# sinamalakouti/CDDMSL

Hardware: AMD Instinct MI355X
Metric: images/sec (train step) VOC+Clipart RN50-C4 (higher is better)
Workload: dtype bf16

## Files before the change

### cddmsl_amd/csrc/conv_fwd.hip

```cpp
#include "gemm_common.h"

namespace {

template <typename T> __device__ __forceinline__ void load8(const char* p, float* f);
template <> __device__ __forceinline__ void load8<__bf16>(const char* p, float* f) {
  const u32x4 v = *(const u32x4*)p;
#pragma unroll
  for (int j = 0; j < 4; ++j) { f[2 * j] = bf2f(v[j] & 0xffff); f[2 * j + 1] = bf2f(v[j] >> 16); }
}
template <> __device__ __forceinline__ void load8<float>(const char* p, float* f) {
  const f32x4 a = ((const f32x4*)p)[0], b = ((const f32x4*)p)[1];
  f[0] = a[0]; f[1] = a[1]; f[2] = a[2]; f[3] = a[3]; f[4] = b[0]; f[5] = b[1]; f[6] = b[2]; f[7] = b[3];
}

__device__ __forceinline__ int swz(int row, int chunk) { return row * KCH + (chunk ^ ((row >> 1) & 7)); }

template <typename T>
__global__ __launch_bounds__(256, 2) void k_conv_fwd_reg(ConvArgs p) {
  __shared__ __attribute__((aligned(16))) u32x4 lds[2][BM * KCH];
  const int t = threadIdx.x;
  const int ntn = (p.Cout + BN - 1) / BN;
  const int tile_n = blockIdx.x % ntn, tile_m = blockIdx.x / ntn;
  const int m0 = tile_m * BM, n0 = tile_n * BN;
  const int cc = t & 7, rb = t >> 3;
// ... 125 lines not shown
#pragma unroll
            for (int j = 0; j < 8; ++j) v[j] = fmaxf(v[j], 0.f);
          }
          if (p.relu_mask) {
            float mv[8];
            load8<T>(p.relu_mask + ((long)m * p.ldm + n) * Mma<T>::ES, mv);
#pragma unroll
            for (int j = 0; j < 8; ++j) if (!(mv[j] > 0.f)) v[j] = 0.f;
          }
          if (p.out_f32 || Mma<T>::ES == 4) {
            f32x4* dst = (f32x4*)(p.y + ((long)m * p.ldy + n) * 4);
            f32x4 o0 = {v[0], v[1], v[2], v[3]}, o1 = {v[4], v[5], v[6], v[7]};
            dst[0] = o0; dst[1] = o1;
          } else {
            u32x4 o = {pack2bf(v[0], v[1]), pack2bf(v[2], v[3]), pack2bf(v[4], v[5]), pack2bf(v[6], v[7])};
            *(u32x4*)(p.y + ((long)m * p.ldy + n) * 2) = o;
          }
        }
      }
    }
    return;
  }
#pragma unroll
  for (int b = 0; b < 2; ++b) {
    int n = n0 + wn * 64 + b * 32 + r;
    if (n >= p.Cout) continue;
    float sc = p.scale ? p.scale[n] : 1.f;
    float bi = p.bias ? p.bias[n] : 0.f;
#pragma unroll
    for (int a = 0; a < 2; ++a) {
#pragma unroll
      for (int g = 0; g < 16; ++g) {
        int m = m0 + wm * 64 + a * 32 + (g & 3) + 8 * (g >> 2) + 4 * h;
        if (m >= p.M) continue;
        float v = affine<T>(acc[a][b][g], sc, bi);
        if (p.residual) v += Mma<T>::load(p.residual + ((long)m * p.ldr + n) * Mma<T>::ES);
        if (p.relu) v = fmaxf(v, 0.f);
        if (p.relu_mask && !(Mma<T>::load(p.relu_mask + ((long)m * p.ldm + n) * Mma<T>::ES) > 0.f)) v = 0.f;
        if (p.out_f32) *(float*)(p.y + ((long)m * p.ldy + n) * 4) = v;
        else Mma<T>::store(p.y + ((long)m * p.ldy + n) * Mma<T>::ES, v);
      }
    }
  }
}


__device__ __forceinline__ long pooled_row(const ConvArgs& p, int m) {
  const unsigned tq = fdiv((unsigned)m, p.dWo), ox = m - tq * p.Wo;
  const unsigned img = fdiv(tq, p.dHo), oy = tq - img * p.Ho;
  const unsigned hp = p.Ho >> 1, wp = p.Wo >> 1;
  return ((oy >> 1) < hp && (ox >> 1) < wp) ? ((long)img * hp + (oy >> 1)) * wp + (ox >> 1) : -1L;
}

template <typename T>
__global__ __launch_bounds__(256, 2) void k_conv_fwd(ConvArgs p) {
  __shared__ __attribute__((aligned(16))) u32x4 lds[2][2][BM * KCH];
  const int t = threadIdx.x;
  p.x += (long)blockIdx.y * p.bx; p.w += (long)blockIdx.y * p.bw; p.y += (long)blockIdx.y * p.by;
  const int wvu = __builtin_amdgcn_readfirstlane(t >> 6);
  const int ntn = (p.Cout + BN - 1) / BN;
  const int lbid = xcd_remap(blockIdx.x, gridDim.x);
  const int tile_n = lbid % ntn, tile_m = lbid / ntn;
  const int m0 = tile_m * BM, n0 = tile_n * BN;
  const int cc = t & 7, rb = t >> 3;
  const int cl = cc ^ ((rb >> 1) & 7);

  long rowoff[4], wrow[4];
  int iy0[4], ix0[4];
  bool vm[4], vn[4];
#pragma unroll
  for (int i = 0; i < 4; ++i) {
    int m = m0 + rb + 32 * i;
    vm[i] = m < p.M;
    unsigned mm = vm[i] ? m : 0;
    unsigned tq = fdiv(mm, p.dWo), ox = mm - tq * p.Wo;
    unsigned img = fdiv(tq, p.dHo), oy = tq - img * p.Ho;
    iy0[i] = (int)oy * p.stride - p.pad;
    ix0[i] = (int)ox * p.stride - p.pad;
    rowoff[i] = ((((long)img * p.Hi + iy0[i]) * p.Wi + ix0[i]) * p.xrs) * 16;
    int n = n0 + rb + 32 * i;
    vn[i] = n < p.Cout;
    wrow[i] = (long)(vn[i] ? n : 0) * p.wrs * 16;
  }
  const int nkt = (p.Kc + KCH - 1) / KCH;
  const char* zp = (const char*)g_zero_page;
  const bool taps = !(p.KH == 1 && p.KW == 1 && p.pad == 0);
  int kc = cl;
  int pp0 = (int)fdiv((unsigned)kc, p.dcpp);
  int coff = kc - pp0 * p.cpp;
  int ky = (int)fdiv((unsigned)pp0, p.dKW), kx = pp0 - ky * p.KW;

  const bool fast = (p.cpp & 7) == 0;
  const char* pa[4];
  const char* pb[4];
  int inca[4], incb[4];
  int tiles_left_in_tap = 0;
  auto retap = [&]() {
    const int delta = ((ky * p.Wi + kx) * p.xrs + coff) * 16;
#pragma unroll
    for (int i = 0; i < 4; ++i) {
      bool ok = vm[i];
      if (taps) {
        int iy = iy0[i] + ky, ix = ix0[i] + kx;
        ok = ok && iy >= 0 && iy < p.Hi && ix >= 0 && ix < p.Wi;
      }
      pa[i] = ok ? p.x + rowoff[i] + delta : zp;
      inca[i] = ok ? KCH * 16 : 0;
    }
  };
  if (fast) {
#pragma unroll
    for (int i = 0; i < 4; ++i) {
      pb[i] = vn[i] ? p.w + wrow[i] + (long)kc * 16 : zp;
      incb[i] = vn[i] ? KCH * 16 : 0;
// ... 344 lines not shown
          *(unsigned short*)(ob + row * (NT * 64) + (nt * 32 + r) * 2) = f2bf(v);
        }
#pragma unroll
      for (int i = 0; i < 2 * NT; ++i) {
        const u32x4 o = *(const u32x4*)(ob + (i * 64 + lane) * 16);
        __builtin_amdgcn_raw_buffer_store_b128(o, ry, (unsigned)((i * 64 + lane) * 16), tile * (32 * NT * 64), 0);
      }
      continue;
    }
    const unsigned vy = (unsigned)(((tile * 32 + 4 * hh) * p.ldy + r) * ES), vmk = (unsigned)(((tile * 32 + 4 * hh) * p.ldm + r) * ES);
#pragma unroll
    for (int nt = 0; nt < NT; ++nt)
#pragma unroll
      for (int g = 0; g < 16; ++g) {
        const int row = (g & 3) + 8 * (g >> 2);
        float v = affine<T>(acc[nt][g], sc[nt], bi[nt]);
        asm("v_max_f32 %0, %1, %2" : "=v"(v) : "v"(v), "s"(relu_floor));
        if (p.relu_mask) {
          float mv;
          if (ES == 2) mv = bf2f((unsigned)__builtin_amdgcn_raw_buffer_load_b16(rm, vmk, (row * p.ldm + nt * 32) * ES, 0));
          else mv = __builtin_bit_cast(float, __builtin_amdgcn_raw_buffer_load_b32(rm, vmk, (row * p.ldm + nt * 32) * ES, 0));
          if (!(mv > 0.f)) v = 0.f;
        }
        if (ES == 2) __builtin_amdgcn_raw_buffer_store_b16((unsigned short)f2bf(v), ry, vy, (row * p.ldy + nt * 32) * ES, 0);
        else __builtin_amdgcn_raw_buffer_store_b32(__builtin_bit_cast(unsigned, v), ry, vy, (row * p.ldy + nt * 32) * ES, 0);
      }
  }
}

template <typename T> void launch_small(const ConvArgs& a, unsigned nb, hipStream_t st) {
  if (a.KH == 1 && a.cpp == 8) hipLaunchKernelGGL((k_conv3x3_small<T, 8, 2, 1>), dim3(nb), dim3(256), 0, st, a);
  else if (a.KH == 1) hipLaunchKernelGGL((k_conv3x3_small<T, 32, 2, 1>), dim3(nb), dim3(256), 0, st, a);
  else if (a.cpp == 1 && a.Cout == 32) hipLaunchKernelGGL((k_conv3x3_small<T, 1, 1>), dim3(nb), dim3(256), 0, st, a);
  else if (a.cpp == 1) hipLaunchKernelGGL((k_conv3x3_small<T, 1, 2>), dim3(nb), dim3(256), 0, st, a);
  else if (a.cpp == 8) hipLaunchKernelGGL((k_conv3x3_small<T, 8, 2>), dim3(nb), dim3(256), 0, st, a);
  else if (a.Cout == 32) hipLaunchKernelGGL((k_conv3x3_small<T, 4, 1>), dim3(nb), dim3(256), 0, st, a);
  else if (a.pool_out) {
    if constexpr (sizeof(T) == 2) hipLaunchKernelGGL((k_conv3x3_small<T, 4, 2, 9, true>), dim3(nb), dim3(256), 0, st, a);
  }
  else hipLaunchKernelGGL((k_conv3x3_small<T, 4, 2>), dim3(nb), dim3(256), 0, st, a);
}

template <typename T> void launch_tile128(const ConvArgs& a, const Plan& p, hipStream_t st) {
  const dim3 grid(p.gx, p.gy);
  switch (p.kernel) {
    case 8: launch_small<T>(a, p.gx, st); break;
    case 2: hipLaunchKernelGGL(k_conv_fwd_reg<T>, grid, dim3(256), 0, st, a); break;
    default: hipLaunchKernelGGL(k_conv_fwd<T>, grid, dim3(256), 0, st, a); break;
  }
}

}

void launch_fwd_tile128(const ConvArgs& a, const Plan& p, Operand op, hipStream_t st) {
  if (op == OP_BF16) launch_tile128<__bf16>(a, p, st);
  else launch_tile128<float>(a, p, st);
}
```

### cddmsl_amd/csrc/conv_fwd256.hip

```cpp
#include "gemm_common.h"
#include <type_traits>

namespace {

__device__ __forceinline__ unsigned pack4_e4m3(float a, float b, float c, float d) {
  a = __builtin_amdgcn_fmed3f(a, -448.f, 448.f); b = __builtin_amdgcn_fmed3f(b, -448.f, 448.f);
  c = __builtin_amdgcn_fmed3f(c, -448.f, 448.f); d = __builtin_amdgcn_fmed3f(d, -448.f, 448.f);
  int w = __builtin_amdgcn_cvt_pk_fp8_f32(a, b, 0, false);
  w = __builtin_amdgcn_cvt_pk_fp8_f32(c, d, w, true);
  return (unsigned)w;
}

struct fp8e4 { unsigned char v; };
template <> struct Mma<fp8e4> {
  static constexpr int ES = 2;
  __device__ static __forceinline__ void step2(f32x16& acc, const u32x4& a0, const u32x4& a1, const u32x4& b0, const u32x4& b1) {
    const i32x8 a = {(int)a0[0], (int)a0[1], (int)a0[2], (int)a0[3], (int)a1[0], (int)a1[1], (int)a1[2], (int)a1[3]};
    const i32x8 b = {(int)b0[0], (int)b0[1], (int)b0[2], (int)b0[3], (int)b1[0], (int)b1[1], (int)b1[2], (int)b1[3]};
    acc = __builtin_amdgcn_mfma_scale_f32_32x32x64_f8f6f4(a, b, acc, 0, 0, 0, 0x7f7f7f7f, 0, 0x7f7f7f7f);
  }
};
template <typename T> struct MmaQuad {
  __device__ static __forceinline__ void run(f32x16& c0, f32x16& c1, const u32x4 (*fa)[4], const u32x4* fb) {
#pragma unroll
// ... 152 lines not shown
#pragma unroll
      for (int j = 0; j < 8; ++j) asm("v_max_f32 %0, %1, %2" : "=v"(v[j]) : "v"(v[j]), "s"(relu_floor));
      if (has_msk) {
        float mv[8];
        if (ES == 2) {
#pragma unroll
          for (int j = 0; j < 4; ++j) { mv[2 * j] = bf2f(rmsk_[i][0][j] & 0xffff); mv[2 * j + 1] = bf2f(rmsk_[i][0][j] >> 16); }
        } else {
#pragma unroll
          for (int j = 0; j < 4; ++j) {
            mv[j] = __builtin_bit_cast(f32x4, rmsk_[i][0])[j]; mv[4 + j] = __builtin_bit_cast(f32x4, rmsk_[i][ES / 2 - 1])[j];
          }
        }
#pragma unroll
        for (int j = 0; j < 8; ++j) if (!(mv[j] > 0.f)) v[j] = 0.f;
      }
      const unsigned so = (unsigned)((a * 32 + 8 * i) * p.ldy * eso);
      if (emit8) {
#pragma unroll
        for (int j = 0; j < 8; ++j) am8 = absmax_bits(am8, v[j]);
        const u32x2 o8 = {pack4_e4m3(v[0] * q8s, v[1] * q8s, v[2] * q8s, v[3] * q8s), pack4_e4m3(v[4] * q8s, v[5] * q8s, v[6] * q8s, v[7] * q8s)};
        __builtin_amdgcn_raw_buffer_store_b64(o8, ry8, vy8, (unsigned)((a * 32 + 8 * i) * p.ldy), CDDMSL_STORE_AUX);
        asm volatile("s_nop 4" ::: "memory");
        asm volatile("" :: "v"(o8));
      }
      if (f32out) {
        const u32x4 o0 = {__builtin_bit_cast(unsigned, v[0]), __builtin_bit_cast(unsigned, v[1]), __builtin_bit_cast(unsigned, v[2]), __builtin_bit_cast(unsigned, v[3])};
        const u32x4 o1 = {__builtin_bit_cast(unsigned, v[4]), __builtin_bit_cast(unsigned, v[5]), __builtin_bit_cast(unsigned, v[6]), __builtin_bit_cast(unsigned, v[7])};
        __builtin_amdgcn_raw_buffer_store_b128(o0, ry, vy, so, CDDMSL_STORE_AUX);
        __builtin_amdgcn_raw_buffer_store_b128(o1, ry, vy, so + 16, CDDMSL_STORE_AUX);
        asm volatile("s_nop 4" ::: "memory");
        asm volatile("" :: "v"(o0), "v"(o1));
      } else {
        const u32x4 o = {pack2bf(v[0], v[1]), pack2bf(v[2], v[3]), pack2bf(v[4], v[5]), pack2bf(v[6], v[7])};
        if (p.nt_out) __builtin_amdgcn_raw_buffer_store_b128(o, ry, vy, so, CDDMSL_STORE_AUX);
        else __builtin_amdgcn_raw_buffer_store_b128(o, ry, vy, so, 0);
        asm volatile("s_nop 4" ::: "memory");
        asm volatile("" :: "v"(o));
      }
    }
    if (DEPTH == 2 && a + 2 < 4 && !rf32) fetch(a + 2, rresb[a % DEPTH], rmskb[a % DEPTH]);
  };
  put(std::integral_constant<int, 0>{});
  pass(std::integral_constant<int, 0>{});
  pass(std::integral_constant<int, 1>{});
  pass(std::integral_constant<int, 2>{});
  pass(std::integral_constant<int, 3>{});
  if (emit8 && p.amax8) {
    am8 = wave_max_u(am8);
    if (lane == 0) atomicMax(p.amax8 + (blockIdx.x & 63), am8);
  }
}

template <typename T, bool TAPS, bool RPOOL = false, int EPI = -1, bool PERSIST = false, bool SPLITK = false>
__global__ __launch_bounds__(512) void k_conv_fwd256(ConvArgs p) {
  __shared__ __attribute__((aligned(16))) u32x4 lds[2 * 2 * 2 * 128 * KCH];
  const int t_in = threadIdx.x;
  p.x += (long)blockIdx.y * p.bx; p.w += (long)blockIdx.y * p.bw; p.y += (long)blockIdx.y * p.by;
  const int ntn = p.Cout >> 8;
  const int ntiles = PERSIST ? (p.tile_limit ? p.tile_limit : ntn * ((p.M + 255) >> 8)) : 0;
  int lbid = PERSIST ? (int)((blockIdx.x & 7) * (gridDim.x >> 3) + (blockIdx.x >> 3))
           : SPLITK ? p.tile0 + (int)(blockIdx.x / (unsigned)p.ksplits) : xcd_remap(blockIdx.x, gridDim.x);
  const int kt0 = SPLITK ? (int)(blockIdx.x % (unsigned)p.ksplits) * p.kper : 0;
  if (PERSIST && lbid >= ntiles) return;
  for (;;) {
  int t = t_in;
  if (PERSIST) asm volatile("" : "+v"(t));
  const int lane = t & 63;
#ifdef CDDMSL_TILE_STAMPS
  const unsigned long long ts_entry = __builtin_amdgcn_s_memrealtime();
#endif
  const int wvu = __builtin_amdgcn_readfirstlane(t >> 6);
  const int wr = wvu >> 2, wc = wvu & 3;
  const int tile_n = lbid % ntn, tile_m = lbid / ntn;
  const int m0 = tile_m * 256, n0 = tile_n * 256;
  const int cl = (t & 7) ^ ((t >> 4) & 7);
  const int nkt = SPLITK ? min(p.kper, (p.Kc >> 3) - kt0) : (p.Kc >> 3);
  const int tpt = p.cpp >> 3;

  auto rowoff = [&](int m, int& iy0, int& ix0) {
    const unsigned tq = fdiv((unsigned)m, p.dWo), ox = m - tq * p.Wo;
    const unsigned img = fdiv(tq, p.dHo), oy = tq - img * p.Ho;
    iy0 = (int)oy * p.stride - p.pad; ix0 = (int)ox * p.stride - p.pad;
    return (((long)img * p.Hi + iy0) * p.Wi + ix0) * p.xrs * 16;
  };
  int iyb, ixb;
  const long base_a = rowoff(m0, iyb, ixb);
  const __amdgpu_buffer_rsrc_t ra_rsrc = __builtin_amdgcn_make_buffer_rsrc((void*)(p.x + base_a), 0, 0x7fffffff, 0x00020000);
  const __amdgpu_buffer_rsrc_t rb_rsrc = __builtin_amdgcn_make_buffer_rsrc((void*)(p.w + (long)n0 * p.wrs * 16), 0, 0x7fffffff, 0x00020000);
  unsigned va[2][2], vinv[2][2], vb[2][2];
  int iy0[2][2], ix0[2][2];
#pragma unroll
  for (int h = 0; h < 2; ++h)
#pragma unroll
    for (int i = 0; i < 2; ++i) {
      const int m = m0 + i * 128 + h * 64 + (t >> 3);
      const bool vm = m < p.M;
      const long ro = rowoff(vm ? m : m0, iy0[h][i], ix0[h][i]);
      va[h][i] = (unsigned)(ro - base_a) + cl * 16;
      if (!vm) { iy0[h][i] = -(1 << 20); if (!TAPS) va[h][i] |= 0x80000000u; }
      vinv[h][i] = 0;
      vb[h][i] = (unsigned)(((2 * i + (t >> 8)) * 64 + h * 32 + ((t >> 3) & 31)) * p.wrs + cl) * 16;
    }
  if (TAPS) {
    unsigned xm[2][2] = {{0, 0}, {0, 0}};
    for (int kx = 0; kx < p.KW; ++kx)
#pragma unroll
      for (int h = 0; h < 2; ++h)
#pragma unroll
        for (int i = 0; i < 2; ++i) xm[h][i] |= ((unsigned)(ix0[h][i] + kx) >= (unsigned)p.Wi ? 1u : 0u) << kx;
    const unsigned full = (1u << p.KW) - 1u;
    for (int ky = 0; ky < p.KH; ++ky)
#pragma unroll
      for (int h = 0; h < 2; ++h)
#pragma unroll
        for (int i = 0; i < 2; ++i) vinv[h][i] |= ((unsigned)(iy0[h][i] + ky) >= (unsigned)p.Hi ? full : xm[h][i]) << (ky * p.KW);
  }
  const int step_col = (p.xrs - (p.cpp - KCH)) * 16;
// ... 126 lines not shown
    readA(I1{}, fa1);
    flipA();
    if (more2) {
      stageB(I0{}, d);
      asm volatile("s_waitcnt vmcnt(4)" ::: "memory");
    } else if (more1) {
      asm volatile("s_waitcnt vmcnt(0)" ::: "memory");
    } else if (PREF) {
      const bool is_res = (EPI & 1) != 0;
      const char* base = is_res ? p.residual : p.relu_mask;
      const int ld = is_res ? p.ldr : p.ldm;
      long bytes = ((long)p.M - m0) * ld * 2;
      if (bytes > 0x7fffffffL) bytes = 0x7fffffffL;
      const __amdgpu_buffer_rsrc_t rs = __builtin_amdgcn_make_buffer_rsrc((void*)(base + (long)m0 * ld * 2), 0, (int)bytes, 0x00020000);
      const unsigned vo = (unsigned)(((wr * 128 + (lane >> 3)) * ld + n0 + wc * 64 + (lane & 7) * 8) * 2);
#pragma unroll
      for (int a = 0; a < 2; ++a)
#pragma unroll
        for (int i = 0; i < 4; ++i) pre[a][i] = __builtin_amdgcn_raw_buffer_load_b128(rs, vo, (a * 32 + 8 * i) * ld * 2, 0);
    }
    CDDMSL_PHASE_SYNC_IN();
    CDDMSL_MMA_QUAD(1, 1, fa1, fb1);
    CDDMSL_PHASE_SYNC_OUT(1, 1);
    if (more1) readA(I0{}, fa0);
    if (more2) stageB(I1{}, d);
    if (last && !SPLITK) {
      const int n = n0 + wc * 64 + (lane & 7) * 8;
      const f32x4 one = {1.f, 1.f, 1.f, 1.f}, zero = {0.f, 0.f, 0.f, 0.f};
      sb[0] = p.scale ? *(const f32x4*)(p.scale + n) : one; sb[1] = p.scale ? *(const f32x4*)(p.scale + n + 4) : one;
      sb[2] = p.bias ? *(const f32x4*)(p.bias + n) : zero; sb[3] = p.bias ? *(const f32x4*)(p.bias + n + 4) : zero;
    }
    CDDMSL_PHASE_SYNC_IN();
    CDDMSL_MMA_QUAD(1, 0, fa1, fb0);
    CDDMSL_PHASE_SYNC_OUT(1, 0);
  };
  for (int kt = 0; kt + 1 < nkt; ++kt) ktile(kt, std::false_type{});
  ktile(nkt - 1, std::true_type{});
  if (wr == 0) __builtin_amdgcn_s_barrier();
#ifdef CDDMSL_TILE_STAMPS
  const unsigned long long ts_epi = __builtin_amdgcn_s_memrealtime();
#endif
#undef CDDMSL_MMA_QUAD
#undef CDDMSL_PHASE_SYNC_IN
#undef CDDMSL_PHASE_SYNC_OUT

  if (SPLITK) {
    store_frags((f32x4*)p.partial + (long)blockIdx.x * (8 * 32 * 64) + (wvu * 32) * 64 + lane, acc);
    return;
  }
  tile_epilogue<T, RPOOL, EPI, PREF>(p, acc, (float*)lds + wvu * 4096, wr, wc, lane, m0, n0, pre, sb);
#ifdef CDDMSL_TILE_STAMPS
  if (p.tstamps && lane == 0) {
    if (!PERSIST) asm volatile("s_waitcnt vmcnt(0)" ::: "memory");
    unsigned long long* o = p.tstamps + ((long)(PERSIST ? lbid : (int)blockIdx.x) * 8 + wvu) * 4;
    o[0] = ts_entry; o[1] = ts_loop; o[2] = ts_epi; o[3] = __builtin_amdgcn_s_memrealtime();
  }
#endif
  if (!PERSIST) break;
  lbid += gridDim.x;
  if (lbid >= ntiles) break;
  __builtin_amdgcn_s_barrier();
  }
}

template <typename T, bool TAPS, int EPI>
__global__ __launch_bounds__(256, 2) void k_conv_fwd2(ConvArgs p) {
  constexpr int SA = 256 * 64, SB = 128 * 64, SS = SA + SB, STAGES = 3;
  __shared__ __attribute__((aligned(16))) u32x4 lds[STAGES * SS / 16];
  const int t = threadIdx.x, lane = t & 63;
#ifdef CDDMSL_TILE_STAMPS
  const unsigned long long ts_entry = __builtin_amdgcn_s_memrealtime();
#endif
  p.x += (long)blockIdx.y * p.bx; p.w += (long)blockIdx.y * p.bw; p.y += (long)blockIdx.y * p.by;
  const int wvu = __builtin_amdgcn_readfirstlane(t >> 6);
  const int wr = wvu >> 1, wc = wvu & 1;
  const int ntn = p.Cout >> 7;
  const int lbid = xcd_remap(blockIdx.x, gridDim.x);
  const int tile_n = lbid % ntn, tile_m = lbid / ntn;
  const int m0 = tile_m * 256, n0 = tile_n * 128;
  const int cl = (t & 3) ^ ((t >> 3) & 3);
  const int nkt = p.Kc >> 2;
  const int tpt = p.cpp >> 2;

  auto rowoff = [&](int m, int& iy0, int& ix0) {
    const unsigned tq = fdiv((unsigned)m, p.dWo), ox = m - tq * p.Wo;
    const unsigned img = fdiv(tq, p.dHo), oy = tq - img * p.Ho;
    iy0 = (int)oy * p.stride - p.pad; ix0 = (int)ox * p.stride - p.pad;
    return (((long)img * p.Hi + iy0) * p.Wi + ix0) * p.xrs * 16;
  };
  int iyb, ixb;
  const long base_a = rowoff(m0, iyb, ixb);
  const __amdgpu_buffer_rsrc_t ra_rsrc = __builtin_amdgcn_make_buffer_rsrc((void*)(p.x + base_a), 0, 0x7fffffff, 0x00020000);
  const __amdgpu_buffer_rsrc_t rb_rsrc = __builtin_amdgcn_make_buffer_rsrc((void*)(p.w + (long)n0 * p.wrs * 16), 0, 0x7fffffff, 0x00020000);
  unsigned va[4], vinv[4], vb[2];
  int iy0[4], ix0[4];
#pragma unroll
  for (int i = 0; i < 4; ++i) {
    const int m = m0 + (t >> 2) + 64 * i;
    const bool vm = m < p.M;
    const long ro = rowoff(vm ? m : m0, iy0[i], ix0[i]);
    va[i] = (unsigned)(ro - base_a) + cl * 16;
    if (!vm) { iy0[i] = -(1 << 20); if (!TAPS) va[i] |= 0x80000000u; }
    vinv[i] = 0;
  }
#pragma unroll
  for (int i = 0; i < 2; ++i) vb[i] = (unsigned)((((t >> 2) + 64 * i) * p.wrs + cl) * 16);
  if (TAPS) {
    unsigned xm[4] = {0, 0, 0, 0};
    for (int kx = 0; kx < p.KW; ++kx)
#pragma unroll
      for (int i = 0; i < 4; ++i) xm[i] |= ((unsigned)(ix0[i] + kx) >= (unsigned)p.Wi ? 1u : 0u) << kx;
    const unsigned full = (1u << p.KW) - 1u;
    for (int ky = 0; ky < p.KH; ++ky)
#pragma unroll
      for (int i = 0; i < 4; ++i) vinv[i] |= ((unsigned)(iy0[i] + ky) >= (unsigned)p.Hi ? full : xm[i]) << (ky * p.KW);
  }
  const int step_col = (p.xrs - (p.cpp - 4)) * 16;
  const int step_row = ((p.Wi - (p.KW - 1)) * p.xrs - (p.cpp - 4)) * 16;
  int left = tpt, tap = 0, kxs = 0;
  unsigned soa = 0, sob = 0;

  char* const L = (char*)lds;
  auto stage = [&](int st) {
    char* dst = L + st * SS + wvu * 1024;
#pragma unroll
    for (int i = 0; i < 4; ++i) {
      unsigned v = va[i];
      if (TAPS) v |= __builtin_amdgcn_ubfe(vinv[i], (unsigned)tap, 1u) << 31;
      blds16(ra_rsrc, v, soa, dst + i * 4096);
    }
// ... 157 lines not shown
  S = (nktot + kper - 1) / kper;
  if (S < 2 || rem * S * 65536 * 4 > ws_bytes) return {};
  return {rem, (int)S, kper};
}

template <typename T, bool TAPS> void launch256_main(const ConvArgs& a, dim3 grid, hipStream_t st, int epi) {
  if constexpr (std::is_same<T, __bf16>::value && !TAPS) {
    const int nb = persistent_blocks();
    if (nb > 0 && grid.y == 1 && (int)grid.x > nb && (a.Kc >> 3) <= env_int("CDDMSL_PERSIST_MAXKT", 8)) {
      with_epi(epi, [&](auto e) { hipLaunchKernelGGL((k_conv_fwd256<T, false, false, decltype(e)::value, true>), dim3(nb), dim3(512), 0, st, a); });
      return;
    }
  }
  with_epi(epi, [&](auto e) { hipLaunchKernelGGL((k_conv_fwd256<T, TAPS, false, decltype(e)::value>), grid, dim3(512), 0, st, a); });
}

template <typename T, bool TAPS> void launch256(const ConvArgs& a, dim3 grid, hipStream_t st, void* ws, long ws_bytes) {
  const int epi = epi_of(a);
  if (sizeof(T) == 4 || epi < 0) { hipLaunchKernelGGL((k_conv_fwd256<T, TAPS, false, -1>), grid, dim3(512), 0, st, a); return; }
  if constexpr (sizeof(T) != 4) {
    if constexpr (std::is_same<T, __bf16>::value) {
      const int tiles = (int)grid.x;
      const TailSplit ts = grid.y == 1 ? plan_tail_split(tiles, persistent_blocks_raw(), a.Kc >> 3, ws ? ws_bytes : 0) : TailSplit{};
      if (ts.splits) {
        ConvArgs m = a, t = a;
        m.tile_limit = tiles - ts.rem;
        launch256_main<T, TAPS>(m, dim3((unsigned)(tiles - ts.rem), 1), st, epi);
        t.partial = (float*)ws; t.tile0 = tiles - ts.rem; t.ksplits = ts.splits; t.kper = ts.kper;
        hipLaunchKernelGGL((k_conv_fwd256<T, TAPS, false, -1, false, true>), dim3((unsigned)(ts.rem * ts.splits)), dim3(512), 0, st, t);
        hipLaunchKernelGGL(k_conv_split_reduce, dim3((unsigned)(ts.rem * 64)), dim3(256), 0, st, t);
        return;
      }
    }
    launch256_main<T, TAPS>(a, grid, st, epi);
  }
}

template <typename T> void launch_tile256(const ConvArgs& a, const Plan& p, hipStream_t st, void* ws, long ws_bytes) {
  const dim3 grid(p.gx, p.gy);
  const bool taps = !(a.KH == 1 && a.KW == 1 && a.pad == 0);
  if constexpr (std::is_same<T, fp8e4>::value) {
    if (taps) launch256<T, true>(a, grid, st, ws, ws_bytes);
    else launch256<T, false>(a, grid, st, ws, ws_bytes);
  } else if (p.kernel == 11) {
    if (taps) launch_fwd2<T, true>(a, grid, st);
    else launch_fwd2<T, false>(a, grid, st);
  } else {
    if (a.res_pool) hipLaunchKernelGGL((k_conv_fwd256<T, false, true>), grid, dim3(512), 0, st, a);
    else if (taps) launch256<T, true>(a, grid, st, ws, ws_bytes);
    else launch256<T, false>(a, grid, st, ws, ws_bytes);
  }
}

}

void launch_fwd_tile256(const ConvArgs& a, const Plan& p, Operand op, hipStream_t st, void* ws, long ws_bytes) {
  if (op == OP_BF16) launch_tile256<__bf16>(a, p, st, ws, ws_bytes);
  else if (op == OP_F32) launch_tile256<float>(a, p, st, ws, ws_bytes);
  else launch_tile256<fp8e4>(a, p, st, ws, ws_bytes);
}
```

### cddmsl_amd/csrc/conv_wgrad.hip

```cpp
#include "gemm_common.h"

namespace {

template <typename T> struct TrFrag;
template <> struct TrFrag<__bf16> {
  __device__ static __forceinline__ u32x4 read(const u32x4* base, int mrow0, int col0, int lane) {
    int g = lane >> 4, li = lane & 15, q = li >> 2, pp = li & 3;
    int hh = g >> 1;
    int col = col0 + 16 * (g & 1) + 4 * pp;
    const char* b = (const char*)base;
    const char* a0 = b + (long)(mrow0 + 8 * hh + q) * (WROW * 16) + col * 2;
    const char* a1 = a0 + 4 * (WROW * 16);
    i16x4 v0 = __builtin_amdgcn_ds_read_tr16_b64_v4i16((__attribute__((address_space(3))) i16x4*)a0);
    i16x4 v1 = __builtin_amdgcn_ds_read_tr16_b64_v4i16((__attribute__((address_space(3))) i16x4*)a1);
    u32x2 p0 = __builtin_bit_cast(u32x2, v0), p1 = __builtin_bit_cast(u32x2, v1);
    u32x4 r = {p0[0], p0[1], p1[0], p1[1]};
    return r;
  }
  static constexpr int MSTEP = 16;
};
template <> struct TrFrag<float> {
  __device__ static __forceinline__ u32x4 read(const u32x4* base, int mrow0, int col0, int lane) {
    int r = lane & 31, hh = lane >> 5;
    const char* b = (const char*)base;
// ... 113 lines not shown
}


template <typename T> struct TrFragS;
template <> struct TrFragS<__bf16> {
  struct Off { int o0, o1; };
  __device__ static __forceinline__ Off prep(int col0, int lane) {
    int g = lane >> 4, li = lane & 15, q = li >> 2, pp = li & 3;
    int hh = g >> 1;
    int ch = ((col0 + 16 * (g & 1)) >> 3) + (pp >> 1);
    int r0 = 8 * hh + q, r1 = r0 + 4;
    Off o;
    o.o0 = r0 * 256 + 16 * (ch ^ fsw(r0)) + 8 * (pp & 1);
    o.o1 = r1 * 256 + 16 * (ch ^ fsw(r1)) + 8 * (pp & 1);
    return o;
  }
  __device__ static __forceinline__ u32x4 read(const u32x4* base, int ms, const Off& o) {
    const unsigned a = (unsigned)(size_t)(const __attribute__((address_space(3))) char*)((const char*)base) + ms * 256;
    u32x2 p0, p1;
    asm volatile("ds_read_b64_tr_b16 %0, %1" : "=v"(p0) : "v"(a + o.o0));
    asm volatile("ds_read_b64_tr_b16 %0, %1" : "=v"(p1) : "v"(a + o.o1));
    u32x4 r = {p0[0], p0[1], p1[0], p1[1]};
    return r;
  }
  static constexpr int MSTEP = 16;
};
template <> struct TrFragS<float> {
  struct Off { int o[4]; };
  __device__ static __forceinline__ Off prep(int col0, int lane) {
    int r = lane & 31, hh = lane >> 5;
    int byte = (col0 + r) * 4;
    Off o;
#pragma unroll
    for (int j = 0; j < 4; ++j) {
      int row = 4 * hh + j;
      o.o[j] = row * 256 + (byte & 15) + 16 * (byte >> 4);
    }
    return o;
  }
  __device__ static __forceinline__ u32x4 read(const u32x4* base, int ms, const Off& o) {
    const char* b = (const char*)base;
    u32x4 v;
#pragma unroll
    for (int j = 0; j < 4; ++j) {
      int off = o.o[j] + ms * 256;
      int row = off >> 8, ch = (off >> 4) & 15;
      v[j] = *(const unsigned int*)(b + (off & ~0xf0) + 16 * (ch ^ fsw(row)));
    }
    return v;
  }
  static constexpr int MSTEP = 8;
};

template <typename T>
__global__ __launch_bounds__(256, 2) void k_conv_wgrad_dma(WgradArgs p) {
  constexpr int ES = Mma<T>::ES;
  constexpr int COLS = 256 / ES;
  __shared__ __attribute__((aligned(16))) u32x4 lds[2][2][WM * 16];
  const int t = threadIdx.x, lane = t & 63, wv = t >> 6;
  p.x += (long)blockIdx.y * p.bx; p.dy += (long)blockIdx.y * p.bd;
  char* outp = (char*)p.dw + (long)blockIdx.y * p.bo;
  const int wvu = __builtin_amdgcn_readfirstlane(t >> 6);
  const int ntn = (p.Cout + COLS - 1) / COLS, ntk = (p.K + COLS - 1) / COLS;
  int bid = xcd_remap(blockIdx.x, gridDim.x);
  const int tile_k = bid % ntk; bid /= ntk;
  const int tile_n = bid % ntn; bid /= ntn;
  const int split = bid;
  const int n0 = tile_n * COLS, k0 = tile_k * COLS;
  const int mt0 = split * p.mtiles_per_split;
  const int total_mt = (p.M + WM - 1) / WM;
  const int mt1 = min(mt0 + p.mtiles_per_split, total_mt);

  const int cc = t & 15, rb = t >> 4;
  const int cl = cc ^ fsw(rb);
  const int kc = k0 * ES / 16 + cl;
  const bool vk = kc < p.Kc;
  const int pp = vk ? kc / p.cpp : 0, coff = vk ? kc - pp * p.cpp : 0;
  const int ky = pp / p.KW, kx = pp - ky * p.KW;
  const int nc = n0 * ES / 16 + cl;
  const bool vn = nc < p.ncc;
  const bool taps = !(p.KH == 1 && p.KW == 1);
  const char* zp = (const char*)g_zero_page;

  int m[4];
  const char* pd[4];
  const char* px[4];
#pragma unroll
  for (int i = 0; i < 4; ++i) {
    m[i] = mt0 * WM + rb + 16 * i;
    pd[i] = p.dy + ((long)m[i] * p.ldd) * ES + (long)nc * 16;
    px[i] = p.x + (((long)m[i] + (long)(ky - p.pad) * p.Wi + (kx - p.pad)) * p.xrs) * 16 + (long)coff * 16;
  }
  const long dstep = (long)WM * p.ldd * ES, xstep = (long)WM * p.xrs * 16;

  auto stage = [&](int buf) {
#pragma unroll
    for (int i = 0; i < 4; ++i) {
      bool vmm = m[i] < p.M;
      glds16((vmm && vn) ? pd[i] : zp, &lds[buf][0][(4 * wvu + 16 * i) * 16]);
    }
#pragma unroll
    for (int i = 0; i < 4; ++i) {
      bool ok = (m[i] < p.M) & vk;
      if (taps) {
        unsigned mm = min((unsigned)m[i], (unsigned)(p.M - 1));
        unsigned tq = fdiv(mm, p.dWo);
        unsigned ox = mm - tq * p.Wo;
        unsigned oy = tq - fdiv(tq, p.dHo) * p.Ho;
        ok = ok & ((unsigned)((int)oy - p.pad + ky) < (unsigned)p.Hi) & ((unsigned)((int)ox - p.pad + kx) < (unsigned)p.Wi);
      }
      glds16(ok ? px[i] : zp, &lds[buf][1][(4 * wvu + 16 * i) * 16]);
    }
#pragma unroll
    for (int i = 0; i < 4; ++i) { m[i] += WM; pd[i] += dstep; px[i] += xstep; }
  };

  constexpr int WT = COLS / 2;
  constexpr int NT = WT / 32;
  const int wn = wv >> 1, wk = wv & 1;
  f32x16 acc[NT][NT];
#pragma unroll
  for (int a = 0; a < NT; ++a)
#pragma unroll
    for (int b = 0; b < NT; ++b)
#pragma unroll
      for (int r = 0; r < 16; ++r) acc[a][b][r] = 0.f;

  typename TrFragS<T>::Off offa[NT], offb[NT];
#pragma unroll
  for (int i = 0; i < NT; ++i) {
    offa[i] = TrFragS<T>::prep(wn * WT + i * 32, lane);
    offb[i] = TrFragS<T>::prep(wk * WT + i * 32, lane);
  }

  if (mt0 < mt1) stage(0);
  for (int mt = mt0; mt < mt1; ++mt) {
    const int cur = (mt - mt0) & 1;
    if (mt + 1 < mt1) {
      stage(cur ^ 1);
      asm volatile("s_waitcnt vmcnt(8)" ::: "memory");
    } else {
      asm volatile("s_waitcnt vmcnt(0)" ::: "memory");
    }
    __builtin_amdgcn_s_barrier();
#pragma unroll
    for (int ms = 0; ms < WM; ms += TrFragS<T>::MSTEP) {
      u32x4 fa[NT], fb[NT];
#pragma unroll
      for (int i = 0; i < NT; ++i) {
        fa[i] = TrFragS<T>::read(lds[cur][0], ms, offa[i]);
        fb[i] = TrFragS<T>::read(lds[cur][1], ms, offb[i]);
      }
      asm volatile("s_waitcnt lgkmcnt(0)" ::: "memory");
      __builtin_amdgcn_sched_barrier(0);
#pragma unroll
      for (int a = 0; a < NT; ++a)
#pragma unroll
        for (int b = 0; b < NT; ++b) Mma<T>::step(acc[a][b], fa[a], fb[b]);
    }
    asm volatile("s_waitcnt lgkmcnt(0)" ::: "memory");
    __builtin_amdgcn_s_barrier();
  }

  const int r = lane & 31, h = lane >> 5;
  if (p.ws) {
    f32x4* dst = (f32x4*)p.ws + ((long)(split * ntn + tile_n) * ntk + tile_k) * (4 * NT * NT * 4 * 64) + (wv * NT * NT * 4) * 64 + lane;
#pragma unroll
    for (int a = 0; a < NT; ++a)
#pragma unroll
      for (int b = 0; b < NT; ++b)
#pragma unroll
        for (int g4 = 0; g4 < 4; ++g4) {
          const f32x4 v = {acc[a][b][4 * g4], acc[a][b][4 * g4 + 1], acc[a][b][4 * g4 + 2], acc[a][b][4 * g4 + 3]};
          dst[((a * NT + b) * 4 + g4) * 64] = v;
        }
    return;
  }
#pragma unroll
  for (int a = 0; a < NT; ++a)
#pragma unroll
    for (int b = 0; b < NT; ++b) {
      int k = k0 + wk * WT + b * 32 + r;
      if (k >= p.K) continue;
#pragma unroll
      for (int g = 0; g < 16; ++g) {
        int n = n0 + wn * WT + a * 32 + (g & 3) + 8 * (g >> 2) + 4 * h;
        if (n >= p.Cout) continue;
        float v = acc[a][b][g] * (p.scale ? p.scale[n] : 1.f);
        long o = (long)n * p.ldo + k;
        if (p.direct == 0) atomicAdd((float*)outp + o, v);
        else if (p.direct == 1) ((float*)outp)[o] = v;
        else Mma<T>::store(outp + o * ES, v);
      }
    }
}

template <typename T>
__global__ __launch_bounds__(256, 2) void k_gemm_tn_stream(WgradArgs p, int nbatch, int bpb) {
  constexpr int ES = Mma<T>::ES;
  constexpr int COLS = 256 / ES;
  __shared__ __attribute__((aligned(16))) u32x4 lds[2][2][WM * 16];
  const int t = threadIdx.x, lane = t & 63, wv = t >> 6;
  const int wvu = __builtin_amdgcn_readfirstlane(t >> 6);
  const int ntk = (p.K + COLS - 1) / COLS;
  const int tile_k = blockIdx.x % ntk, tile_n = blockIdx.x / ntk;
  const int n0 = tile_n * COLS, k0 = tile_k * COLS;
  const int b0 = blockIdx.y * bpb, nb = min(bpb, nbatch - b0);
  const int nmt = (p.M + WM - 1) / WM;
  const int nit = nb * nmt;

  const int cc = t & 15, rb = t >> 4;
  const int cl = cc ^ fsw(rb);
  const int kc = k0 * ES / 16 + cl, nc = n0 * ES / 16 + cl;
  const bool vk = kc < p.Kc, vn = nc < p.ncc;
  const char* zp = (const char*)g_zero_page;
  int sb = 0, smt = 0;
  auto stage = [&](int buf) {
    const char* db = p.dy + (long)(b0 + sb) * p.bd + (long)nc * 16;
    const char* xb = p.x + (long)(b0 + sb) * p.bx + (long)kc * 16;
// ... 218 lines not shown
        for (int g = 0; g < 16; ++g) {
          const int n0 = a * 32 + (g & 3) + 8 * (g >> 2);
          const bool exists = a * 4 + (g >> 2) < NG;
          const bool lo_ok = n0 >= 1 && n0 <= P, hi_ok = n0 + 4 >= 1 && n0 + 4 <= P;
          if (exists) {
            const int n = n0 + 4 * h;
            const float v = acc[a][g];
            gacc[a][g] += (n == 0) ? t0 : v;
            if (lo_ok || hi_ok) {
              if (h ? hi_ok : lo_ok) {
                const unsigned word = (n - 1) < 32 ? mlo : mhi;
                const bool keep = (word >> ((n - 1) & 31)) & 1u;
                Mma<__bf16>::store(outp + ((long)(n - 1) * p.ldo + k) * 2, keep ? v + base : 0.f);
              }
            }
          }
          acc[a][g] = 0.f;
        }
      return;
    }
#pragma unroll
    for (int a = 0; a < NTN; ++a)
#pragma unroll
      for (int g = 0; g < 16; ++g) {
        if (a * 4 + (g >> 2) < NG) {
          const int n = a * 32 + (g & 3) + 8 * (g >> 2) + 4 * h;
          const float v = acc[a][g];
          const long o = (long)n * p.ldo + k;
          if (MODE == 0) atomicAdd((float*)outp + o, v);
          else if (MODE == 1) ((float*)outp)[o] = v;
          else Mma<__bf16>::store(outp + o * 2, v);
        }
        acc[a][g] = 0.f;
      }
  };
  {
    int it = 0;
    for (; it + 2 < nit; ++it) item(it, std::integral_constant<int, 2>{});
    if (it + 1 < nit) { item(it, std::integral_constant<int, 1>{}); ++it; }
    if (it < nit) item(it, std::integral_constant<int, 0>{});
  }
  if (MODE == 3 && p.gpos) {
    const int k = k0 + wvu * 32 + r;
#pragma unroll
    for (int a = 0; a < NTN; ++a)
#pragma unroll
      for (int g = 0; g < 16; ++g) {
        const int n = a * 32 + (g & 3) + 8 * (g >> 2) + 4 * h;
        if (a * 4 + (g >> 2) < NG && n <= P) atomicAdd(p.gpos + (long)n * p.K + k, gacc[a][g]);
      }
  }
}

__global__ __launch_bounds__(512) void k_wgrad256(WgradArgs p) {
  __shared__ __attribute__((aligned(16))) u32x4 lds[2 * 2 * 2 * 64 * 16];
  const int t = threadIdx.x, lane = t & 63;
#ifdef CDDMSL_TILE_STAMPS
  const unsigned long long ts_entry = __builtin_amdgcn_s_memrealtime();
  unsigned long long ts_loop = ts_entry;
#endif
  p.x += (long)blockIdx.y * p.bx; p.dy += (long)blockIdx.y * p.bd;
  char* outp = (char*)p.dw + (long)blockIdx.y * p.bo;
  const int wvu = __builtin_amdgcn_readfirstlane(t >> 6);
  const int wn = wvu >> 2, wk = wvu & 3;
  const int ntn = p.Cout >> 8, ntk = p.K >> 8;
  int bid = xcd_remap(blockIdx.x, gridDim.x);
  const int tile_k = bid % ntk; bid /= ntk;
  const int tile_n = bid % ntn; bid /= ntn;
  const int n0 = tile_n * 256, k0 = tile_k * 256;
  const int mt0 = bid * p.mtiles_per_split;
  const int nmt = min(p.mtiles_per_split, (p.M + WM - 1) / WM - mt0);
  const bool taps = !(p.KH == 1 && p.KW == 1);

  const int rb = t >> 4, cl = (t & 15) ^ fsw(rb);
  const int gd = (cl >> 3) * 16 + (cl & 7);
  const int gx = (cl >> 2) * 8 + (cl & 3);
  const int kc = (k0 >> 3) + gx;
  const int pp = kc / p.cpp, coff = kc - pp * p.cpp;
  const int ky = pp / p.KW, kx = pp - ky * p.KW;
  unsigned vd[2], vx[2];
#pragma unroll
  for (int i = 0; i < 2; ++i) {
    vd[i] = (unsigned)((i * 32 + rb) * p.ldd * 2 + gd * 16);
    vx[i] = (unsigned)((((i * 32 + rb) + ky * p.Wi + kx) * p.xrs + coff) * 16);
  }
  const __amdgpu_buffer_rsrc_t rd = __builtin_amdgcn_make_buffer_rsrc((void*)(p.dy + ((long)mt0 * WM * p.ldd + n0) * 2), 0, 0x80000000u, 0x00020000);
  const __amdgpu_buffer_rsrc_t rx = __builtin_amdgcn_make_buffer_rsrc((void*)(p.x + ((long)mt0 * WM - p.pad * p.Wi - p.pad) * p.xrs * 16), 0, 0x80000000u, 0x00020000);
  const unsigned dstep = (unsigned)(WM * p.ldd * 2), xstep = (unsigned)(WM * p.xrs * 16);
  const int mrow = mt0 * WM + rb;

  char* const L = (char*)lds;
  auto stageD = [&](auto H, int buf, int T) {
    constexpr int h = decltype(H)::value;
    char* dst = L + (buf << 16) + (h << 14) + wvu * 1024;
#pragma unroll
    for (int i = 0; i < 2; ++i) {
      const unsigned inv = (mrow + T * WM + i * 32 < p.M) ? 0u : 0x80000000u;
      __builtin_amdgcn_raw_ptr_buffer_load_lds(rd, (__attribute__((address_space(3))) void*)(dst + i * 8192 - h * 128), 16,
                                               (int)(vd[i] | inv), (int)(T * dstep), h * 128, 0);
    }
  };
  unsigned xinv[2];
  auto validX = [&](int T) {
#pragma unroll
    for (int i = 0; i < 2; ++i) {
      const int m = mrow + T * WM + i * 32;
      bool ok = m < p.M;
      if (taps) {
        const unsigned mm = min((unsigned)m, (unsigned)(p.M - 1));
        const unsigned tq = fdiv(mm, p.dWo);
        const unsigned ox = mm - tq * p.Wo;
        const unsigned oy = tq - fdiv(tq, p.dHo) * p.Ho;
        ok = ok & ((unsigned)((int)oy - p.pad + ky) < (unsigned)p.Hi) & ((unsigned)((int)ox - p.pad + kx) < (unsigned)p.Wi);
      }
      xinv[i] = ok ? 0u : 0x80000000u;
    }
  };
  auto stageX = [&](auto J, int buf, int T) {
    constexpr int j = decltype(J)::value;
    char* dst = L + (buf << 16) + (1 << 15) + (j << 14) + wvu * 1024;
#pragma unroll
// ... 82 lines not shown
#ifdef CDDMSL_TILE_STAMPS
    ts_loop = __builtin_amdgcn_s_memrealtime();
#endif

    for (int kt = 0; kt < nmt; ++kt) {
      const int d = kt & 1;
      const bool more1 = kt + 1 < nmt, more2 = kt + 2 < nmt;
      CDDMSL_READ_B(0, fb0)
      if (more1) stageD(I1{}, d ^ 1, kt + 1);
      CDDMSL_PHASE_SYNC_IN(CDDMSL_WAIT4(fb0))
      CDDMSL_MMA_QUAD(0, 0, fa0, fb0);
      CDDMSL_PHASE_SYNC_OUT(0, 0)
      CDDMSL_READ_B(1, fb1)
      CDDMSL_FLIP_B()
      if (more2) { stageD(I0{}, d, kt + 2); validX(kt + 2); }
      CDDMSL_PHASE_SYNC_IN(CDDMSL_WAIT4(fb1))
      CDDMSL_MMA_QUAD(0, 1, fa0, fb1);
      CDDMSL_PHASE_SYNC_OUT(0, 1)
      CDDMSL_READ_A(1, fa1)
      CDDMSL_FLIP_A()
      if (more2) {
        stageX(I0{}, d, kt + 2);
        asm volatile("s_waitcnt vmcnt(4)" ::: "memory");
      } else {
        asm volatile("s_waitcnt vmcnt(0)" ::: "memory");
      }
      CDDMSL_PHASE_SYNC_IN(CDDMSL_WAIT8(fa1))
      CDDMSL_MMA_QUAD(1, 1, fa1, fb1);
      CDDMSL_PHASE_SYNC_OUT(1, 1)
      if (more1) { CDDMSL_READ_A(0, fa0) }
      if (more2) stageX(I1{}, d, kt + 2);
      CDDMSL_PHASE_SYNC_IN(CDDMSL_WAIT8(fa0))
      CDDMSL_MMA_QUAD(1, 0, fa1, fb0);
      CDDMSL_PHASE_SYNC_OUT(1, 0)
    }
    if (wn == 0) __builtin_amdgcn_s_barrier();
  }
#undef CDDMSL_TR2
#undef CDDMSL_WAIT4
#undef CDDMSL_WAIT8
#undef CDDMSL_READ_A
#undef CDDMSL_READ_B
#undef CDDMSL_FLIP_A
#undef CDDMSL_FLIP_B
#undef CDDMSL_MMA_QUAD
#undef CDDMSL_PHASE_SYNC_IN
#undef CDDMSL_PHASE_SYNC_OUT

#ifdef CDDMSL_TILE_STAMPS
  const unsigned long long ts_epi = __builtin_amdgcn_s_memrealtime();
#endif
  const int r = lane & 31, h = lane >> 5;
  if (p.ws) {
    store_frags((f32x4*)p.ws + ((long)(bid * ntn + tile_n) * ntk + tile_k) * (8 * 32 * 64) + (wvu * 32) * 64 + lane, acc);
  } else
#pragma unroll
  for (int a = 0; a < 4; ++a)
#pragma unroll
    for (int b = 0; b < 2; ++b) {
      const int k = k0 + wk * 64 + b * 32 + r;
#pragma unroll
      for (int g = 0; g < 16; ++g) {
        const int n = n0 + wn * 128 + a * 32 + (g & 3) + 8 * (g >> 2) + 4 * h;
        const float v = acc[a][b][g] * (p.scale ? p.scale[n] : 1.f);
        const long o = (long)n * p.ldo + k;
        if (p.direct == 0) atomicAdd((float*)outp + o, v);
        else if (p.direct == 1) ((float*)outp)[o] = v;
        else Mma<__bf16>::store(outp + o * 2, v);
      }
    }
#ifdef CDDMSL_TILE_STAMPS
  if (p.tstamps && lane == 0) {
    asm volatile("s_waitcnt vmcnt(0)" ::: "memory");
    unsigned long long* o = p.tstamps + ((long)blockIdx.x * 8 + wvu) * 4;
    o[0] = ts_entry; o[1] = ts_loop; o[2] = ts_epi; o[3] = __builtin_amdgcn_s_memrealtime();
  }
#endif
}

__global__ __launch_bounds__(512) void k_wgrad256_f8(WgradArgs p) {
  __shared__ __attribute__((aligned(16))) u32x4 lds[4 * 2 * 64 * 16];
  const int t = threadIdx.x, lane = t & 63;
  const int wvu = __builtin_amdgcn_readfirstlane(t >> 6);
  const int wn = wvu >> 2, wk = wvu & 3;
  const int ntn = p.Cout >> 8, ntk = p.K >> 8;
  int bid = xcd_remap(blockIdx.x, gridDim.x);
  const int tile_k = bid % ntk; bid /= ntk;
  const int tile_n = bid % ntn; bid /= ntn;
  const int n0 = tile_n * 256, k0 = tile_k * 256;
  const int mt0 = bid * p.mtiles_per_split;
  const int nmt_real = min(p.mtiles_per_split, (p.M + WM - 1) / WM - mt0);
  const int nmt = (nmt_real + 1) & ~1;
  const int mlim = min(p.M, (mt0 + nmt_real) * WM);
  const bool taps = !(p.KH == 1 && p.KW == 1);

  const int rq = lane >> 4, r8 = (wvu & 1) * 4 + rq;
  const int cl = (lane & 15) ^ (r8 << 1);
  const int pp = k0 / p.Cin, coff = (k0 - pp * p.Cin) >> 4;
  const int ky = pp / p.KW, kx = pp - ky * p.KW;
  unsigned vd[2], vx[2];
#pragma unroll
  for (int i = 0; i < 2; ++i) {
    const int row = i * 32 + wvu * 4 + rq;
    vd[i] = (unsigned)(row * p.ldd + cl * 16);
    vx[i] = (unsigned)(((row + ky * p.Wi + kx) * p.xrs + coff + cl) * 16);
  }
  const __amdgpu_buffer_rsrc_t rd = __builtin_amdgcn_make_buffer_rsrc((void*)(p.dy + ((long)mt0 * WM * p.ldd + n0)), 0, 0x80000000u, 0x00020000);
// ... 135 lines not shown
#pragma unroll
      for (int g = 0; g < 16; ++g) {
        const int n = n0 + wn * 128 + a * 32 + (g & 3) + 8 * (g >> 2) + 4 * h;
        atomicAdd(p.dw + (long)n * p.ldo + k, acc[a][b][g] * (p.scale ? p.scale[n] : 1.f));
      }
    }
}

}

template <int WAVES, int FR>
__global__ __launch_bounds__(256) void k_wgrad_reduce(const f32x4* ws, float* dw, const float* scale, int ntn, int ntk, int splits, int Cout, int K, int ldo) {
  constexpr int SLOTS = WAVES * FR * 64;
  constexpr int TN = WAVES == 8 ? 256 : 128;
  const int tile = blockIdx.x / (SLOTS / 256), q = (blockIdx.x % (SLOTS / 256)) * 256 + threadIdx.x;
  const int tile_k = tile % ntk, tile_n = tile / ntk;
  const long ntiles = (long)ntn * ntk;
  const f32x4* src = ws + (long)tile * SLOTS + q;
  f32x4 sum = {0.f, 0.f, 0.f, 0.f};
  int s = 0;
  for (; s + 4 <= splits; s += 4) {
    const f32x4 a = src[(s + 0) * ntiles * SLOTS], b = src[(s + 1) * ntiles * SLOTS], c = src[(s + 2) * ntiles * SLOTS], d = src[(s + 3) * ntiles * SLOTS];
    sum += (a + b) + (c + d);
  }
  for (; s < splits; ++s) sum += src[s * ntiles * SLOTS];
  const int wv = q / (FR * 64), j = (q / 64) % FR, lane = q & 63, r = lane & 31, h = lane >> 5, g4 = j & 3;
  int a, b, wn, wk;
  if (WAVES == 8) { a = j >> 3; b = (j >> 2) & 1; wn = wv >> 2; wk = wv & 3; }
  else { a = j >> 3; b = (j >> 2) & 1; wn = wv >> 1; wk = wv & 1; }
  const int n = tile_n * TN + wn * (WAVES == 8 ? 128 : 64) + a * 32 + 8 * g4 + 4 * h;
  const int k = tile_k * TN + wk * 64 + b * 32 + r;
  if (k >= K) return;
#pragma unroll
  for (int e = 0; e < 4; ++e)
    if (n + e < Cout) dw[(long)(n + e) * ldo + k] += sum[e] * (scale ? scale[n + e] : 1.f);
}

static bool use_workspace(long blocks, long tile_floats, void* ws, long ws_bytes) {
  if (env_int("CDDMSL_WGRAD_WS", 1) == 0) return false;
  return ws != nullptr && blocks * tile_floats * 4 <= ws_bytes;
}

template <int WAVES, int FR>
static void launch_wgrad_split(void (*kernel)(WgradArgs), WgradArgs& a, const Plan& p, hipStream_t st, void* wsp, long ws_bytes) {
  constexpr int TN = WAVES == 8 ? 256 : 128, SLOTS = WAVES * FR * 64;
  const int ntn = (a.Cout + TN - 1) / TN, ntk = (a.K + TN - 1) / TN;
  const bool ws = p.splits > 1 && use_workspace((long)p.gx, SLOTS * 4, wsp, ws_bytes);
  if (ws) a.ws = (float*)wsp;
  hipLaunchKernelGGL(kernel, dim3(p.gx), dim3(WAVES * 64), 0, st, a);
  if (ws) hipLaunchKernelGGL((k_wgrad_reduce<WAVES, FR>), dim3((unsigned)(ntn * ntk * (SLOTS / 256))), dim3(256), 0, st, (const f32x4*)wsp, a.dw, a.scale,
                             ntn, ntk, p.splits, a.Cout, a.K, a.ldo);
}

void launch_wgrad(WgradArgs& a, const Plan& p, Operand op, hipStream_t st, void* ws, long ws_bytes) {
  switch (p.kernel) {
    case 12: launch_wgrad_split<8, 32>(k_wgrad256_f8, a, p, st, ws, ws_bytes); break;
    case 6: launch_wgrad_split<8, 32>(k_wgrad256, a, p, st, ws, ws_bytes); break;
    case 5:
      if (op == OP_BF16) launch_wgrad_split<4, 16>(k_conv_wgrad_dma<__bf16>, a, p, st, ws, ws_bytes);
      else hipLaunchKernelGGL(k_conv_wgrad_dma<float>, dim3(p.gx), dim3(256), 0, st, a);
      break;
    default:
      if (op == OP_BF16) hipLaunchKernelGGL(k_conv_wgrad<__bf16>, dim3(p.gx), dim3(256), 0, st, a);
      else hipLaunchKernelGGL(k_conv_wgrad<float>, dim3(p.gx), dim3(256), 0, st, a);
  }
}

void launch_gemm_tn(const WgradArgs& p, Operand op, const Plan& pl, int batch, int mode, hipStream_t st) {
  const dim3 grid(pl.gx, pl.gy);
  if (pl.kernel == 9) {
#define CDDMSL_TNS(NG)                                                                                              \
  case NG:                                                                                                          \
    if (mode == 0) hipLaunchKernelGGL((k_gemm_tn_small<NG, 0>), grid, dim3(256), 0, st, p, batch, pl.bpb);      \
    else if (mode == 1) hipLaunchKernelGGL((k_gemm_tn_small<NG, 1>), grid, dim3(256), 0, st, p, batch, pl.bpb); \
    else hipLaunchKernelGGL((k_gemm_tn_small<NG, 2>), grid, dim3(256), 0, st, p, batch, pl.bpb);                \
    break;
    switch (p.Cout / 8) { CDDMSL_TNS(1) CDDMSL_TNS(2) CDDMSL_TNS(3) CDDMSL_TNS(4) CDDMSL_TNS(5) CDDMSL_TNS(6) CDDMSL_TNS(7) CDDMSL_TNS(8) }
#undef CDDMSL_TNS
  } else if (pl.kernel == 7) {
    if (op == OP_BF16) hipLaunchKernelGGL(k_gemm_tn_stream<__bf16>, grid, dim3(256), 0, st, p, batch, pl.bpb);
    else hipLaunchKernelGGL(k_gemm_tn_stream<float>, grid, dim3(256), 0, st, p, batch, pl.bpb);
  } else {
    if (op == OP_BF16) hipLaunchKernelGGL(k_conv_wgrad_dma<__bf16>, grid, dim3(256), 0, st, p);
    else hipLaunchKernelGGL(k_conv_wgrad_dma<float>, grid, dim3(256), 0, st, p);
  }
}

void launch_attnpool_dx(const WgradArgs& p, unsigned gx, unsigned gy, int nbatch, int bpb, hipStream_t st) {
  hipLaunchKernelGGL((k_gemm_tn_small<7, 3, 49>), dim3(gx, gy), dim3(256), 0, st, p, nbatch, bpb);
}
```

### cddmsl_amd/csrc/gemm_common.h

```cpp
#pragma once
#include "common.h"
#include <cstdlib>

namespace {

constexpr int BM = 128, BN = 128, KCH = 8;

struct FastDiv {
  unsigned mul, shr, d;
};
static inline FastDiv make_fastdiv(unsigned d) {
  FastDiv f;
  f.d = d;
  unsigned s = 0;
  while ((1ull << s) < d) ++s;
  f.shr = s;
  f.mul = (unsigned)(((1ull << 32) * ((1ull << s) - d)) / d + 1);
  return f;
}
__device__ __forceinline__ unsigned fdiv(unsigned n, const FastDiv& f) { return (__umulhi(n, f.mul) + n) >> f.shr; }

template <typename T> __device__ __forceinline__ float affine(float v, float sc, float bi) {
  return sizeof(T) <= 2 ? __builtin_fmaf(v, sc, bi) : v * sc + bi;
}

#ifndef CDDMSL_STORE_AUX
#define CDDMSL_STORE_AUX 2
#endif
#ifndef CDDMSL_LOAD_AUX
#define CDDMSL_LOAD_AUX 0
#endif

struct ConvArgs {
  const char* x;
  const char* w;
  char* y;
  const float* scale;
  const float* bias;
  const char* residual;
  const char* relu_mask;
  int Nimg, Hi, Wi, Cin, Ho, Wo, Cout, KH, KW, stride, pad;
  int ldy, ldr, ldm;
  int relu, out_f32, pool;
  int res_f32;
  int res_pool;
  int M, Kc, cpp;
  FastDiv dWo, dHo, dcpp, dKW;
  int xrs, wrs;
  long bx, bw, by;
  char* y8 = nullptr;
  const float* q8 = nullptr;
  unsigned* amax8 = nullptr;
  float* partial = nullptr;
  int tile0 = 0, ksplits = 1, kper = 0, tile_limit = 0;
  int pool_out = 0;
  FastDiv dWp = {}, dHp = {};
  int nt_out = 1;
#ifdef CDDMSL_TILE_STAMPS
  unsigned long long* tstamps = nullptr;
#endif
};

template <typename T> struct Mma;
template <> struct Mma<__bf16> {
  static constexpr int ES = 2;
  __device__ static __forceinline__ void step(f32x16& acc, const u32x4& a, const u32x4& b) {
    acc = __builtin_amdgcn_mfma_f32_32x32x16_bf16(__builtin_bit_cast(bf16x8, a), __builtin_bit_cast(bf16x8, b), acc, 0, 0, 0);
  }
  __device__ static __forceinline__ float load(const char* p) { return bf2f(*(const unsigned short*)p); }
  __device__ static __forceinline__ void store(char* p, float v) { *(unsigned short*)p = f2bf(v); }
};
template <> struct Mma<float> {
  static constexpr int ES = 4;
  __device__ static __forceinline__ void step(f32x16& acc, const u32x4& a, const u32x4& b) {
    const f32x4 fa = __builtin_bit_cast(f32x4, a), fb = __builtin_bit_cast(f32x4, b);
    acc = __builtin_amdgcn_mfma_f32_32x32x2f32(fa[0], fb[0], acc, 0, 0, 0);
    acc = __builtin_amdgcn_mfma_f32_32x32x2f32(fa[1], fb[1], acc, 0, 0, 0);
    acc = __builtin_amdgcn_mfma_f32_32x32x2f32(fa[2], fb[2], acc, 0, 0, 0);
    acc = __builtin_amdgcn_mfma_f32_32x32x2f32(fa[3], fb[3], acc, 0, 0, 0);
  }
  __device__ static __forceinline__ float load(const char* p) { return *(const float*)p; }
  __device__ static __forceinline__ void store(char* p, float v) { *(float*)p = v; }
};
typedef __attribute__((ext_vector_type(8))) int i32x8;

__device__ __forceinline__ int xcd_remap(int bid, int nblk) {
  const int q = nblk >> 3, rem = nblk & 7, x = bid & 7, j = bid >> 3;
  return (x < rem ? x * (q + 1) : rem * (q + 1) + (x - rem) * q) + j;
}

template <typename T> __device__ __forceinline__ u32x4 avg4(const u32x4& a, const u32x4& b, const u32x4& c, const u32x4& d);
template <> __device__ __forceinline__ u32x4 avg4<float>(const u32x4& a, const u32x4& b, const u32x4& c, const u32x4& d) {
  const f32x4 fa = __builtin_bit_cast(f32x4, a), fb = __builtin_bit_cast(f32x4, b);
  const f32x4 fc = __builtin_bit_cast(f32x4, c), fd = __builtin_bit_cast(f32x4, d);
  f32x4 r = ((fa + fb) + (fc + fd)) * 0.25f;
  return __builtin_bit_cast(u32x4, r);
}
template <> __device__ __forceinline__ u32x4 avg4<__bf16>(const u32x4& a, const u32x4& b, const u32x4& c, const u32x4& d) {
  u32x4 r;
#pragma unroll
  for (int j = 0; j < 4; ++j) {
    float lo = (bf2f(a[j] & 0xffff) + bf2f(b[j] & 0xffff)) + (bf2f(c[j] & 0xffff) + bf2f(d[j] & 0xffff));
    float hi = (bf2f(a[j] >> 16) + bf2f(b[j] >> 16)) + (bf2f(c[j] >> 16) + bf2f(d[j] >> 16));
    r[j] = pack2bf(lo * 0.25f, hi * 0.25f);
  }
  return r;
}

__device__ __attribute__((aligned(16))) unsigned int g_zero_page[4] = {0u, 0u, 0u, 0u};

__device__ __forceinline__ void glds16(const void* g, void* l) {
  __builtin_amdgcn_global_load_lds((const __attribute__((address_space(1))) void*)g,
                                   (__attribute__((address_space(3))) void*)l, 16, 0, 0);
}

struct WgradArgs {
  const char* x;
  const char* dy;
  float* dw;
  const float* scale;
  int Nimg, Hi, Wi, Cin, Ho, Wo, Cout, KH, KW, stride, pad, ldd, pool;
  int M, Kc, cpp, K, ncc;
  int mtiles_per_split;
  FastDiv dWo, dHo;
  int xrs;
  int ldo;
  int direct;
  long bx, bd, bo;
  const float* g0 = nullptr;
  const unsigned long long* mbits = nullptr;
  float* gpos = nullptr;
  float* ws = nullptr;
#ifdef CDDMSL_TILE_STAMPS
  unsigned long long* tstamps = nullptr;
#endif
};

constexpr int WM = 64;
constexpr int WROW = 16 + 4;

__device__ __forceinline__ int fsw(int row) { return ((row & 3) << 2) | ((row >> 2) & 3); }

__device__ __forceinline__ void store_frags(f32x4* dst, const f32x16 (&acc)[4][2]) {
#pragma unroll
  for (int a = 0; a < 4; ++a)
#pragma unroll
    for (int b = 0; b < 2; ++b)
#pragma unroll
      for (int g4 = 0; g4 < 4; ++g4) {
        const f32x4 v = {acc[a][b][4 * g4], acc[a][b][4 * g4 + 1], acc[a][b][4 * g4 + 2], acc[a][b][4 * g4 + 3]};
        dst[((a * 2 + b) * 4 + g4) * 64] = v;
      }
}

static long env_int(const char* name, long dflt, bool* set = nullptr) {
  const char* e = getenv(name);
  if (set) *set = e != nullptr;
  return e ? atol(e) : dflt;
}

enum Operand { OP_BF16 = 0, OP_F32 = 1, OP_FP8 = 2 };
static int elem_size(Operand op) { return op == OP_BF16 ? 2 : op == OP_F32 ? 4 : 1; }

struct Plan {
  int kernel;
  unsigned gx, gy;
  int splits;
  int mtiles_per_split;
  int bpb;
};

static int persistent_blocks_raw() {
  static int ncu = -1;
  if (ncu < 0) {
    int dev = 0, n = 0;
    if (hipGetDevice(&dev) != hipSuccess || hipDeviceGetAttribute(&n, hipDeviceAttributeMultiprocessorCount, dev) != hipSuccess) n = 0;
    ncu = (n / 8) * 8;
  }
  return ncu;
}

}

extern "C" {
__attribute__((visibility("hidden"))) void launch_fwd_tile128(const ConvArgs& a, const Plan& p, Operand op, hipStream_t st);
__attribute__((visibility("hidden"))) void launch_fwd_tile256(const ConvArgs& a, const Plan& p, Operand op, hipStream_t st, void* ws, long ws_bytes);
__attribute__((visibility("hidden"))) void launch_wgrad(WgradArgs& a, const Plan& p, Operand op, hipStream_t st, void* ws, long ws_bytes);
__attribute__((visibility("hidden"))) void launch_gemm_tn(const WgradArgs& p, Operand op, const Plan& pl, int batch, int mode, hipStream_t st);
__attribute__((visibility("hidden"))) void launch_attnpool_dx(const WgradArgs& p, unsigned gx, unsigned gy, int nbatch, int bpb, hipStream_t st);
__attribute__((visibility("hidden"))) bool record_kernel(int id);
}
```

### cddmsl_amd/csrc/gemm_conv.hip

```cpp
#include "gemm_common.h"

namespace {

template <typename T>
__device__ __forceinline__ void weight_prep_body(const float* w, const float* scale, char* wf, char* wd, int Cout, int KH, int KW, int Cin,
                                                 long first, long stride) {
  __shared__ float tile[32][33];
  const int taps = KH * KW, nit = (Cin + 31) / 32, nct = (Cout + 31) / 32;
  const long ntiles = (long)nct * taps * nit;
  const int tx = threadIdx.x & 31, ty = threadIdx.x >> 5;
  constexpr int ES = Mma<T>::ES;
  for (long tl = first; tl < ntiles; tl += stride) {
    const int it = (int)(tl % nit); const long q = tl / nit;
    const int tap = (int)(q % taps), ct = (int)(q / taps);
    const int ky = tap / KW, kx = tap % KW;
    __syncthreads();
#pragma unroll
    for (int r = 0; r < 4; ++r) {
      const int co = ct * 32 + ty + 8 * r, ci = it * 32 + tx;
      float v = 0.f;
      if (co < Cout && ci < Cin) {
        const long i = ((long)co * taps + tap) * Cin + ci;
        v = w[i];
        if (wf) Mma<T>::store(wf + i * ES, v);
// ... 117 lines not shown
  if ((Cin * es) % 16 != 0) return CDDMSL_ERR_ARG;
  if (pool && (KH != 1 || KW != 1 || pad != 0 || stride != 1)) return CDDMSL_ERR_ARG;
  a.x = (const char*)x; a.w = (const char*)w; a.y = (char*)y; a.scale = scale; a.bias = bias;
  a.residual = (const char*)residual; a.relu_mask = (const char*)relu_mask;
  a.Nimg = Nimg; a.Hi = Hi; a.Wi = Wi; a.Cin = Cin; a.Cout = Cout; a.KH = KH; a.KW = KW; a.stride = stride; a.pad = pad;
  if (pool) { a.Ho = Hi / 2; a.Wo = Wi / 2; }
  else { a.Ho = (Hi + 2 * pad - KH) / stride + 1; a.Wo = (Wi + 2 * pad - KW) / stride + 1; }
  if (a.Ho <= 0 || a.Wo <= 0) return CDDMSL_ERR_ARG;
  if ((out_f32 & 2) && (!(out_f32 & 1) || !residual || relu_mask || pool)) return CDDMSL_ERR_ARG;
  a.ldy = ldy; a.ldr = ldr; a.ldm = ldm; a.relu = relu; a.out_f32 = out_f32 & 1; a.pool = pool;
  a.res_f32 = (op == OP_BF16 && (out_f32 & 2)) ? 1 : 0;
  a.res_pool = (out_f32 & 4) ? 1 : 0;
  if (a.res_pool && (!residual || (out_f32 & 2) || pool || KH != 1 || KW != 1 || pad != 0 || (long)Nimg * (a.Ho / 2) * (a.Wo / 2) * ldr * es >= (1L << 31) ||
                     (Cout & 7) || (ldy & 7) || (ldr & 7) || (relu_mask && (ldm & 7)))) return CDDMSL_ERR_ARG;
  if (a.res_f32 && ((Cout & 7) || (ldy & 7) || (ldr & 7))) return CDDMSL_ERR_ARG;
  long M = (long)Nimg * a.Ho * a.Wo;
  if (M > 0x7fffff00L) return CDDMSL_ERR_ARG;
  a.M = (int)M; a.cpp = Cin * es / 16; a.Kc = KH * KW * a.cpp;
  a.dWo = make_fastdiv((unsigned)a.Wo); a.dHo = make_fastdiv((unsigned)a.Ho);
  a.dcpp = make_fastdiv((unsigned)a.cpp); a.dKW = make_fastdiv((unsigned)KW);
  a.xrs = a.cpp; a.wrs = a.Kc; a.bx = a.bw = a.by = 0;
#ifdef CDDMSL_TILE_STAMPS
  a.tstamps = g_tile_stamps;
#endif
  if (a.M == 0) return CDDMSL_OK;
  a.nt_out = nt_out_for((long)a.M * Cout * 2);
  if (y8) {
    if (op == OP_F32 || (out_f32 & 1) || ldy != Cout) return CDDMSL_ERR_ARG;
    a.y8 = (char*)y8; a.q8 = q8; a.amax8 = (unsigned*)amax8;
  }
  return CDDMSL_OK;
}

static int conv_fwd_any(Operand op, const void* x, const void* w, void* y, const float* scale, const float* bias,
                        const void* residual, const void* relu_mask, int Nimg, int Hi, int Wi, int Cin,
                        int Cout, int KH, int KW, int stride, int pad, int pool, int ldy, int ldr, int ldm,
                        int relu, int out_f32, void* y8, const float* q8, float* amax8, void* stream) {
  ConvArgs a;
  const int st = fill_conv(a, op, x, w, y, scale, bias, residual, relu_mask, Nimg, Hi, Wi, Cin, Cout, KH, KW, stride, pad, pool, ldy, ldr, ldm,
                           relu, out_f32, y8, q8, amax8);
  if (st != CDDMSL_OK || a.M == 0) return st;
  return run_fwd(a, op, plan_fwd(a, op, 1), stream);
}

extern "C" int cddmsl_conv_fwd(const void* x, const void* w, void* y, const float* scale, const float* bias,
                               const void* residual, const void* relu_mask, int Nimg, int Hi, int Wi, int Cin,
                               int Cout, int KH, int KW, int stride, int pad, int pool, int ldy, int ldr, int ldm,
                               int relu, int out_f32, int dtype, void* stream) {
  if (dtype != 0 && dtype != 1) return CDDMSL_ERR_ARG;
  return conv_fwd_any((Operand)dtype, x, w, y, scale, bias, residual, relu_mask, Nimg, Hi, Wi, Cin, Cout, KH, KW, stride, pad, pool, ldy, ldr, ldm,
                      relu, out_f32, nullptr, nullptr, nullptr, stream);
}

extern "C" int cddmsl_conv3x3_pool_fwd(const void* x, const void* w, void* y, const float* scale, const float* bias, const void* relu_mask,
                                       int Nimg, int Hi, int Wi, int Cin, int Cout, int stride, int dtype, void* stream) {
  if (dtype != 0 || Cin != 32 || Cout != 64 || stride != 1 || relu_mask || !scale || !bias || Hi < 2 || Wi < 2) return CDDMSL_ERR_ARG;
  ConvArgs a;
  const int st = fill_conv(a, OP_BF16, x, w, y, scale, bias, nullptr, nullptr, Nimg, Hi, Wi, Cin, Cout, 3, 3, 1, 1, 0, Cout, 0, 0, 1, 0,
                           nullptr, nullptr, nullptr);
  if (st != CDDMSL_OK || a.M == 0) return st;
  if ((long)Nimg * Hi * Wi * Cin * 2 >= 0x7ffff000L || (long)Nimg * (a.Ho / 2) * (a.Wo / 2) * Cout * 2 >= 0x7fffffffL) return CDDMSL_ERR_ARG;
  a.pool_out = 1;
  a.dWp = make_fastdiv((unsigned)(a.Wo / 2)); a.dHp = make_fastdiv((unsigned)(a.Ho / 2));
  const Plan pl = plan_fwd(a, OP_BF16, 1);
  if (pl.kernel != 8) return CDDMSL_ERR_ARG;
  return run_fwd(a, OP_BF16, pl, stream);
}

extern "C" int cddmsl_conv_fwd_q8(const void* x, const void* w, void* y, const float* scale, const float* bias,
                                  const void* residual, const void* relu_mask, int Nimg, int Hi, int Wi, int Cin,
                                  int Cout, int KH, int KW, int stride, int pad, int relu, void* y8, const float* q8, float* amax8,
                                  void* stream) {
  if (!y8) return CDDMSL_ERR_ARG;
  return conv_fwd_any(OP_BF16, x, w, y, scale, bias, residual, relu_mask, Nimg, Hi, Wi, Cin, Cout, KH, KW, stride, pad, 0, Cout, Cout, Cout,
                      relu, 0, y8, q8, amax8, stream);
}

extern "C" int cddmsl_conv_fwd_fp8(const void* x, const void* w, void* y, const float* scale, const float* bias,
                                   const void* residual, const void* relu_mask, int Nimg, int Hi, int Wi, int Cin, int Cout, int KH,
                                   int KW, int pad, int relu, int out_f32, void* y8, const float* q8, float* amax8, void* stream) {
  if (Cin % 128 != 0 || (out_f32 & ~1)) return CDDMSL_ERR_ARG;
  return conv_fwd_any(OP_FP8, x, w, y, scale, bias, residual, relu_mask, Nimg, Hi, Wi, Cin, Cout, KH, KW, 1, pad, 0, Cout, Cout, Cout,
                      relu, out_f32, y8, q8, amax8, stream);
}

static bool wgrad256_ok(const WgradArgs& a, int batch) {
  const long mode = env_int("CDDMSL_GEMM256", 1);
  if (mode == 0) return false;
  if ((a.Cout & 255) || (a.K & 255) || (a.cpp & 7) || (a.ldd & 7)) return false;
  if (mode == 2) return true;
  return (long)(a.Cout / 256) * (a.K / 256) * batch * ((a.M + WM - 1) / WM) >= env_int("CDDMSL_WGRAD256_MIN", 4000);
}
static bool wgrad256_span_ok(int mtiles_per_split, int Wi, long row_bytes) {
  return ((long)mtiles_per_split * WM + WM + 2L * Wi + 2) * row_bytes + (1L << 20) < (1L << 31);
}

static int even_split(int total_mt, long* splits) {
  const int mps = (int)((total_mt + *splits - 1) / *splits);
  *splits = (total_mt + mps - 1) / mps;
  return mps;
}

static long split_512_rounds(long tiles, int total_mt, bool taps) {
  bool forced;
  const long target = env_int("CDDMSL_WGRAD_BLOCKS", taps ? 1024 : 512, &forced);
  const long maxs = (total_mt + 7) / 8;
// ... 59 lines not shown
  }
  return {same ? 5 : 4, (unsigned)(tiles * splits), 1, (int)splits, mps};
}

extern "C" int cddmsl_set_workspace(void* ptr, long bytes) {
  if (bytes < 0 || (ptr == nullptr && bytes != 0) || ((size_t)ptr & 15)) return CDDMSL_ERR_ARG;
  g_ws = ptr; g_ws_bytes = bytes;
  return CDDMSL_OK;
}

static int run_wgrad(WgradArgs& a, Operand op, const Plan& p, void* stream) {
  if (p.kernel == 0) return CDDMSL_ERR_ARG;
  g_last_kernel = p.kernel;
  if (g_plan_only) return CDDMSL_OK;
  a.mtiles_per_split = p.mtiles_per_split;
  launch_wgrad(a, p, op, (hipStream_t)stream, g_ws, g_ws_bytes);
  return launch_status();
}

static int fill_wgrad(WgradArgs& a, Operand op, const void* x, const void* dy, float* dw, const float* scale, int Nimg, int Hi,
                      int Wi, int Cin, int Cout, int KH, int KW, int stride, int pad, int pool, int ldd) {
  const int es = elem_size(op);
  if (Nimg < 0 || Hi <= 0 || Wi <= 0 || Cin <= 0 || Cout <= 0 || KH <= 0 || KW <= 0 || stride <= 0) return CDDMSL_ERR_ARG;
  if ((Cin * es) % 16 != 0 || (Cout * es) % 16 != 0 || (ldd * es) % 16 != 0) return CDDMSL_ERR_ARG;
  if (pool && (KH != 1 || KW != 1 || pad != 0 || stride != 1)) return CDDMSL_ERR_ARG;
  a.x = (const char*)x; a.dy = (const char*)dy; a.dw = dw; a.scale = scale;
  a.Nimg = Nimg; a.Hi = Hi; a.Wi = Wi; a.Cin = Cin; a.Cout = Cout; a.KH = KH; a.KW = KW; a.stride = stride; a.pad = pad;
  a.ldd = ldd; a.pool = pool;
  if (pool) { a.Ho = Hi / 2; a.Wo = Wi / 2; }
  else { a.Ho = (Hi + 2 * pad - KH) / stride + 1; a.Wo = (Wi + 2 * pad - KW) / stride + 1; }
  if (a.Ho <= 0 || a.Wo <= 0) return CDDMSL_ERR_ARG;
  long M = (long)Nimg * a.Ho * a.Wo;
  if (M > 0x7fffff00L) return CDDMSL_ERR_ARG;
  a.M = (int)M; a.cpp = Cin * es / 16; a.Kc = KH * KW * a.cpp; a.K = KH * KW * Cin; a.ncc = Cout * es / 16;
  a.mtiles_per_split = 0;
  a.dWo = make_fastdiv((unsigned)a.Wo); a.dHo = make_fastdiv((unsigned)a.Ho);
  a.xrs = a.cpp; a.ldo = a.K; a.direct = 0; a.bx = a.bd = a.bo = 0;
#ifdef CDDMSL_TILE_STAMPS
  a.tstamps = g_tile_stamps;
#endif
  return CDDMSL_OK;
}

extern "C" int cddmsl_conv_wgrad(const void* x, const void* dy, float* dw, const float* scale, int Nimg, int Hi,
                                 int Wi, int Cin, int Cout, int KH, int KW, int stride, int pad, int pool, int ldd,
                                 int dtype, void* stream) {
  if (dtype != 0 && dtype != 1) return CDDMSL_ERR_ARG;
  WgradArgs a;
  const int st = fill_wgrad(a, (Operand)dtype, x, dy, dw, scale, Nimg, Hi, Wi, Cin, Cout, KH, KW, stride, pad, pool, ldd);
  if (st != CDDMSL_OK || a.M == 0) return st;
  return run_wgrad(a, (Operand)dtype, plan_wgrad(a, (Operand)dtype, 1), stream);
}

extern "C" int cddmsl_conv_wgrad_fp8_ok(int Cin, int Cout, int KH, int KW, int pad, int ldd) {
  return (Cin % 256 == 0 && Cout % 256 == 0 && KH == KW && (KH & 1) && 2 * pad == KH - 1 && ldd % 16 == 0) ? 1 : 0;
}
extern "C" int cddmsl_conv_wgrad_fp8(const void* x8, const void* dy8, float* dw, const float* scale, int Nimg, int Hi, int Wi, int Cin,
                                     int Cout, int KH, int KW, int pad, int ldd, void* stream) {
  if (!cddmsl_conv_wgrad_fp8_ok(Cin, Cout, KH, KW, pad, ldd) || ldd < Cout) return CDDMSL_ERR_ARG;
  WgradArgs a;
  const int st = fill_wgrad(a, OP_FP8, x8, dy8, dw, scale, Nimg, Hi, Wi, Cin, Cout, KH, KW, 1, pad, 0, ldd);
  if (st != CDDMSL_OK || a.M == 0) return st;
  return run_wgrad(a, OP_FP8, plan_wgrad(a, OP_FP8, 1), stream);
}

extern "C" int cddmsl_gemm_nt_batched(const void* a, const void* w, void* c, const float* bias, int M, int N, int K, int lda,
                                      int ldb, int ldc, int batch, long sa, long sw, long sc, int out_f32, int dtype, void* stream) {
  int es = dtype == 0 ? 2 : 4;
  if (dtype != 0 && dtype != 1) return CDDMSL_ERR_ARG;
  if (M < 0 || N <= 0 || K <= 0 || batch < 0 || batch > 65535) return CDDMSL_ERR_ARG;
  if ((K * es) % 16 || (lda * es) % 16 || (ldb * es) % 16 || (sa * es) % 16 || (sw * es) % 16) return CDDMSL_ERR_ARG;
  if (M == 0 || batch == 0) return CDDMSL_OK;
  const Operand op = (Operand)dtype;
  ConvArgs p;
  const int st = fill_conv(p, op, a, w, c, nullptr, bias, nullptr, nullptr, 1, 1, M, K, N, 1, 1, 1, 0, 0, ldc, 0, 0, 0, out_f32 ? 1 : 0,
                           nullptr, nullptr, nullptr);
  if (st != CDDMSL_OK) return st;
  p.xrs = lda * es / 16; p.wrs = ldb * es / 16;
  p.bx = sa * es; p.bw = sw * es; p.by = sc * (out_f32 ? 4 : es);
  p.nt_out = 1;
  return run_fwd(p, op, plan_fwd(p, op, batch), stream);
}

static unsigned tn_small_grid(long kt, long batch, int* bpb) {
  long b = (kt * batch + 4095) / 4096;
  if (b < 8) b = 8;
  if (b > batch) b = batch;
  *bpb = (int)b;
  return (unsigned)((batch + b - 1) / b);
}

static Plan plan_gemm_tn(const WgradArgs& p, Operand op, int batch, int mode) {
  const int cols = 256 / elem_size(op), M = p.M, N = p.Cout, K = p.K;
  const long tiles = (long)((N + cols - 1) / cols) * ((K + cols - 1) / cols);
  const int total_mt = (M + WM - 1) / WM;
  if (op == OP_BF16 && total_mt == 1 && N <= 64 && batch >= 64 && K % 128 == 0 && N % 8 == 0) {
    Plan p = {9, (unsigned)(K / 128), 0};
    p.gy = tn_small_grid(K / 128, batch, &p.bpb);
    return p;
  }
  if (total_mt <= 4 && batch >= 64) {
    long bpb = (tiles * batch + 4095) / 4096, minb = (8 + total_mt - 1) / total_mt;
    if (bpb < minb) bpb = minb;
    if (bpb > batch) bpb = batch;
    return {7, (unsigned)tiles, (unsigned)((batch + bpb - 1) / bpb), 0, 0, (int)bpb};
  }
// ... 69 lines not shown
```

### cddmsl_amd/hip.py

```python
import ctypes
import math
import os
from ctypes import c_float, c_int, c_long, c_void_p

import torch

from ._lib import check, lib, ptr, require_cuda, stream_ptr

DT = {torch.bfloat16: 0, torch.float32: 1}

_sigs_done = False


def _L():
    global _sigs_done
    L = lib()
    if not _sigs_done:
        vp, ci, cf = c_void_p, c_int, c_float
        L.cddmsl_last_kernel.argtypes = []
        L.cddmsl_plan_only.argtypes = [ci]
        L.cddmsl_conv_fwd.argtypes = [vp] * 7 + [ci] * 16 + [vp]
        L.cddmsl_bottleneck64_ok.argtypes = [ci] * 4
        L.cddmsl_bottleneck64_fwd.argtypes = [vp] * 17 + [ci] * 4 + [vp]
        L.cddmsl_conv_wgrad.argtypes = [vp] * 4 + [ci] * 12 + [vp]
        L.cddmsl_set_workspace.argtypes = [vp, c_long]
        L.cddmsl_weight_prep.argtypes = [vp] * 4 + [ci] * 5 + [vp]
        L.cddmsl_weight_prep_multi.argtypes = [vp, ci, ci, vp]
        L.cddmsl_preprocess.argtypes = [vp, vp] + [ci] * 6 + [vp, vp, ci, ci, vp]
        L.cddmsl_maxpool3s2_fwd.argtypes = [vp, vp] + [ci] * 5 + [vp]
        L.cddmsl_upsample_zero2.argtypes = [vp] * 4 + [ci] * 5 + [vp]
        L.cddmsl_meanpool_fwd.argtypes = [vp, vp, c_long, ci, ci, ci, vp]
        L.cddmsl_meanpool_bwd.argtypes = [vp, vp, c_long, ci, ci, ci, vp]
        L.cddmsl_preprocess224.argtypes = [vp, vp] + [ci] * 11 + [vp, vp, ci, vp]
        L.cddmsl_preprocess_batch.argtypes = [vp, vp, vp, ci, vp, ci, ci, ci, vp, vp, ci, ci, vp]
        L.cddmsl_preprocess224_batch.argtypes = [vp, vp, vp, ci, vp] + [ci] * 8 + [vp, vp, ci, vp]
        L.cddmsl_tta_view.argtypes = [vp] + [ci] * 4 + [vp, vp, vp, ci] * 2 + [vp, ci, ci, ci] * 2 + [ci, vp, vp, ci, ci, vp]
        L.cddmsl_avgpool2_fwd.argtypes = [vp, vp] + [ci] * 5 + [vp]
        L.cddmsl_avgpool2_bwd.argtypes = [vp] * 4 + [ci] * 5 + [vp]
        L.cddmsl_avgpool2_bwd_q8.argtypes = [vp] * 4 + [ci] * 4 + [vp] * 4
        L.cddmsl_avgpool2_fwd_bits.argtypes = [vp] * 3 + [ci] * 5 + [vp]
        L.cddmsl_avgpool2_bwd_bits.argtypes = [vp] * 3 + [ci] * 5 + [vp]
        L.cddmsl_conv3x3_pool_fwd.argtypes = [vp] * 6 + [ci] * 7 + [vp]
        L.cddmsl_attn_tokens_fwd.argtypes = [vp] * 3 + [ci] * 5 + [vp]
        L.cddmsl_attn_tokens_bwd.argtypes = [vp] * 4 + [ci] * 5 + [vp]
        L.cddmsl_attnpool_softmax_fwd.argtypes = [vp] * 3 + [c_long, ci, ci, ci, cf, ci, vp]
        L.cddmsl_attnpool_softmax_bwd.argtypes = [vp] * 4 + [c_long, ci, ci, ci, cf, ci, vp]
        L.cddmsl_gemm_nt_batched.argtypes = [vp] * 4 + [ci] * 7 + [c_long] * 3 + [ci, ci, vp]
        L.cddmsl_gemm_tn_batched.argtypes = [vp] * 3 + [ci] * 7 + [c_long] * 3 + [ci, ci, vp]
        L.cddmsl_relu_bwd.argtypes = [vp, vp, vp, c_long, ci, ci, vp]
        L.cddmsl_colsum.argtypes = [vp, vp, c_long, ci, ci, ci, vp]
        L.cddmsl_sgd_clip_step.argtypes = [vp] * 4 + [ci, vp] + [cf] * 4 + [ci, vp]
        L.cddmsl_roi_align_forward.argtypes = [vp] * 5 + [ci] * 7 + [cf, ci, ci, ci, vp]
        L.cddmsl_roi_align_backward.argtypes = [vp] * 7 + [ci] * 7 + [cf, ci, ci, ci, vp]
        L.cddmsl_nms_anyorder.argtypes = [vp] * 4 + [ci, cf, vp, vp, vp]
        L.cddmsl_soft_nms.argtypes = [vp] * 6 + [ci, ci, cf, cf, cf, ci, vp, vp, vp]
        L.cddmsl_openset_logits.argtypes = [vp] * 4 + [ci] * 4 + [cf, cf, vp]
        L.cddmsl_openset_select.argtypes = [vp, vp, ci, vp, ci, vp, ci, ci, cf, cf, cf] + [vp] * 6 + [ci, vp, vp, vp]
        L.cddmsl_roi_align_nchw_anyorder.argtypes = [vp] * 3 + [ci] * 7 + [cf, ci, ci, ci, vp, vp, vp]
        L.cddmsl_roi_align_backward_nchw_anyorder.argtypes = [vp] * 3 + [ci] * 7 + [cf, ci, ci, ci, vp, vp, vp]
        L.cddmsl_quantize_fp8.argtypes = [vp] * 4 + [c_long, ci, vp]
        L.cddmsl_conv_fwd_fp8.argtypes = [vp] * 7 + [ci] * 10 + [vp] * 4
        L.cddmsl_conv_wgrad_fp8_ok.argtypes = [ci] * 6
        L.cddmsl_conv_wgrad_fp8.argtypes = [vp] * 4 + [ci] * 9 + [vp]
        L.cddmsl_conv_fwd_q8.argtypes = [vp] * 7 + [ci] * 10 + [vp] * 4
        L.cddmsl_fp8_dot_nt.argtypes = [vp] * 4 + [ci] * 4 + [vp]
        L.cddmsl_roi_align_forward_affine.argtypes = [vp] * 6 + [ci] * 8 + [cf, ci, ci, ci] + [vp] * 4
        L.cddmsl_roi_align_backward_pooled.argtypes = [vp] * 7 + [ci] * 7 + [cf, ci, ci, ci, vp]
        L.cddmsl_anchors.argtypes = [vp, vp, ci, ci, ci, cf, cf, vp]
        L.cddmsl_sort_desc.argtypes = [vp] * 5 + [ci, ci, vp, vp, vp]
        L.cddmsl_rpn_decode.argtypes = [vp] * 6 + [ci] * 5 + [cf] * 8 + [vp]
        L.cddmsl_nms.argtypes = [vp] * 5 + [ci, ci, cf, ci, vp]
        L.cddmsl_iou_match.argtypes = [vp, ci, vp, ci, vp, vp, vp, ci, cf, cf, ci, ci, ci, ci, vp]
        L.cddmsl_iou_match_batched.argtypes = [vp] * 7 + [ci] * 5 + [cf, cf] + [ci] * 4 + [vp]
        L.cddmsl_l2norm_fwd.argtypes = [vp, vp, vp, c_long, ci, cf, vp]
        L.cddmsl_l2norm_bwd.argtypes = [vp, vp, vp, vp, c_long, ci, vp]
        L.cddmsl_cosine_logits_fwd.argtypes = [vp] * 4 + [c_long, ci, ci, cf, cf, vp]
        L.cddmsl_cosine_logits_bwd.argtypes = [vp] * 5 + [c_long, ci, ci, cf, ci, vp]
# ... 142 lines not shown
    N, H, W, Cin = x.shape
    Cout, KH, KW, Cin2 = w.shape
    assert Cin == Cin2, (x.shape, w.shape)
    if pool:
        Ho, Wo = H // 2, W // 2
    else:
        Ho, Wo = (H + 2 * pad - KH) // stride + 1, (W + 2 * pad - KW) // stride + 1
    ydt = torch.float32 if out_f32 else x.dtype
    if out_spec is not None and out_spec.full is None:
        out_spec.full = torch.empty((2 * N, Ho, Wo, Cout), device=x.device, dtype=ydt)
        y, out_spec.used = out_spec.full[:N], 1
    elif out_spec is not None and out_spec.used == 1 and tuple(out_spec.full.shape) == (2 * N, Ho, Wo, Cout) and out_spec.full.dtype == ydt:
        y, out_spec.used = out_spec.full[N:], 2
    else:
        y = torch.empty((N, Ho, Wo, Cout), device=x.device, dtype=ydt)
    for v in (scale, bias):
        assert v is None or (v.dtype == torch.float32 and v.numel() == Cout and v.is_contiguous())
    res_f32 = residual is not None and residual.dtype == torch.float32 and x.dtype != torch.float32
    if res_f32:
        assert out_f32 and relu_mask is None and not pool and Cout % 8 == 0
    if residual_pooled:
        assert residual is not None and not res_f32 and residual.dtype == x.dtype and residual.is_contiguous()
        assert tuple(residual.shape) == (N, Ho // 2, Wo // 2, Cout) and pooled_residual_ok(residual), residual.shape
    for v in (residual, relu_mask):
        assert v is None or (v is residual and residual_pooled) or (
            (v.dtype == x.dtype or (v is residual and res_f32)) and v.is_contiguous() and v.numel() == y.numel())
    y8 = None
    if emit8 is not None:
        assert x.dtype == torch.bfloat16 and not out_f32 and not pool and not residual_pooled and not res_f32
        y8 = torch.empty(y.shape, device=x.device, dtype=torch.uint8)

    def launch():
        if y8 is not None:
            return _L().cddmsl_conv_fwd_q8(ptr(x), ptr(w), ptr(y), ptr(scale), ptr(bias), ptr(residual), ptr(relu_mask),
                                           N, H, W, Cin, Cout, KH, KW, stride, pad, int(relu), ptr(y8), ptr(emit8[0]), ptr(emit8[1]), stream_ptr())
        return _L().cddmsl_conv_fwd(ptr(x), ptr(w), ptr(y), ptr(scale), ptr(bias), ptr(residual), ptr(relu_mask),
                                    N, H, W, Cin, Cout, KH, KW, stride, pad, int(pool), Cout, Cout, Cout,
                                    int(relu), int(out_f32) | (2 if res_f32 else 0) | (4 if residual_pooled else 0), _dt(x), stream_ptr())
    e0 = PROFILE.begin(plan=launch) if PROFILE.on else None
    st = launch()
    check(st, "cddmsl_conv_fwd")
    PROFILE.end(e0, _CONV_KERNEL.get(_L().cddmsl_last_kernel(), "conv_fwd") if e0 is not None else "conv_fwd",
                2.0 * N * Ho * Wo * Cout * KH * KW * Cin,
                (N * Ho * Wo, Cout, KH * KW * Cin, KH, int(pool), stride),
                nbytes=float(_conv_input_pixels(N, H, W, Ho, Wo, KH, KW, stride, bool(pool)) * Cin * x.element_size()
                             + w.numel() * w.element_size() + y.numel() * y.element_size()
                             + (residual.numel() * residual.element_size() if residual is not None else 0)
                             + (relu_mask.numel() * relu_mask.element_size() if relu_mask is not None else 0)))
    if y8 is not None:
        y._fp8 = (y8, emit8[0].data_ptr())
    return y


def conv3x3_pool_fwd(x, w, scale, bias, relu_mask=None, stride=1):
    require_cuda(x, w, scale, bias, relu_mask)
    assert x.dim() == 4 and w.dim() == 4 and x.is_contiguous() and w.is_contiguous() and x.dtype == w.dtype
    N, H, W, Cin = x.shape
    Cout, KH, KW, Cin2 = w.shape
    assert (KH, KW, Cin2) == (3, 3, Cin), (x.shape, w.shape)
    for v in (scale, bias):
        assert v is not None and v.dtype == torch.float32 and v.numel() == Cout and v.is_contiguous()
    assert relu_mask is None or (relu_mask.dtype == x.dtype and relu_mask.is_contiguous())
    y = torch.empty((N, H // 2, W // 2, Cout), device=x.device, dtype=x.dtype)

    def launch():
        return _L().cddmsl_conv3x3_pool_fwd(ptr(x), ptr(w), ptr(y), ptr(scale), ptr(bias), ptr(relu_mask), N, H, W, Cin, Cout, stride,
                                            _dt(x), stream_ptr())
    e0 = PROFILE.begin(plan=launch) if PROFILE.on else None
    check(launch(), "cddmsl_conv3x3_pool_fwd")
    Mc = N * (H // 2) * (W // 2) * 4
    PROFILE.end(e0, "k_conv3x3_small", 2.0 * Mc * Cout * 9 * Cin, (Mc, Cout, 9 * Cin, 3, 2, 1),
                nbytes=float(x.numel() * x.element_size() + w.numel() * w.element_size() + y.numel() * y.element_size()))
    return y


def bottleneck64_ok(o1, w2, w3, wd=None, w1n=None):
    if not (o1.is_cuda and o1.dtype == torch.bfloat16 and o1.dim() == 4 and o1.is_contiguous() and o1.shape[3] == 64):
        return False
    want = ((w2, (64, 3, 3, 64)), (w3, (256, 1, 1, 64)), (wd, (256, 1, 1, 64)), (w1n, (64, 1, 1, 256)))
    if any(w is not None and (tuple(w.shape) != s or w.dtype != torch.bfloat16 or not w.is_contiguous()) for w, s in want):
        return False
    N, H, W, _ = o1.shape
    return N > 0 and bool(_L().cddmsl_bottleneck64_ok(N, H, W, 0))


def bottleneck64_fwd(o1, w2, bn2, w3, bn3, residual=None, x0=None, wd=None, bnd=None, w1n=None, bn1n=None):
    require_cuda(o1, w2, w3, residual, x0, wd, w1n)
    assert bottleneck64_ok(o1, w2, w3, wd, w1n) and (residual is None) != (wd is None)
    N, H, W, _ = o1.shape
    for t, c in ((residual, 256), (x0 if wd is not None else None, 64)):
        assert t is None or (t.dtype == torch.bfloat16 and t.is_contiguous() and tuple(t.shape) == (N, H, W, c))
    for bn, c in ((bn2, 64), (bn3, 256), (bnd, 256), (bn1n, 64)):
        assert bn is None or all(v.dtype == torch.float32 and v.numel() == c and v.is_contiguous() and v.is_cuda for v in bn)
    assert (wd is None) == (bnd is None) and (w1n is None) == (bn1n is None) and (wd is None or x0 is not None)
    out = torch.empty((N, H, W, 256), device=o1.device, dtype=o1.dtype)
    o1n = torch.empty((N, H, W, 64), device=o1.device, dtype=o1.dtype) if w1n is not None else None
    sd, bd = bnd if bnd is not None else (None, None)
    s1n, b1n = bn1n if bn1n is not None else (None, None)
    e0 = PROFILE.begin(name="k_bottleneck64") if PROFILE.on else None
    check(_L().cddmsl_bottleneck64_fwd(ptr(o1), ptr(w2), ptr(bn2[0]), ptr(bn2[1]), ptr(w3), ptr(bn3[0]), ptr(bn3[1]), ptr(residual),
                                       ptr(x0 if wd is not None else None), ptr(wd), ptr(sd), ptr(bd), ptr(w1n), ptr(s1n), ptr(b1n),
                                       ptr(out), ptr(o1n), N, H, W, 0, stream_ptr()), "cddmsl_bottleneck64_fwd")
    M = N * H * W
    kn = 576 * 64 + 64 * 256 + (64 * 256 if wd is not None else 0) + (256 * 64 if w1n is not None else 0)
    PROFILE.end(e0, "k_bottleneck64", 2.0 * M * kn, (M, 256, 576, 3, int(wd is not None), int(w1n is not None)),
                nbytes=float(2 * M * (64 + (64 if wd is not None else 256) + 256 + (64 if w1n is not None else 0)) + 2 * kn))
# ... 1334 lines not shown
```

### cddmsl_amd/layers.py

```python
import os
import weakref

import torch

from . import hip

_STEP = [0]


def bump_weight_version():
    _STEP[0] += 1


_LOAD_GEN = [0]


def note_weights_loaded(*_):
    _LOAD_GEN[0] += 1
    _STEP[0] += 1


def load_generation():
    return _LOAD_GEN[0]

# ... 515 lines not shown
        dpre2 = dgrad_auto(gs, bp.pw[2], f8, gs_slot, emit8=e8, relu_mask=o2)
    dpre1 = dgrad_auto(dpre2, bp.pw[1], f8, d2_slot, pad=1, relu_mask=o1, emit8=d1_slot.emit() if d1_slot is not None else None)
    wgrad_auto(o1, dpre2, bp.pw[1], s2, 1, _ohwi(_grad_buf(w2p)), f8, o1_8, d2_slot)
    if d1_slot is not None:
        wgrad_auto(x, dpre1, bp.pw[0], s1, 0, _ohwi(_grad_buf(w1p)), f8, x8, d1_slot, taps_only=False)
    else:
        hip.conv_wgrad(x, dpre1, shp(w1p), s1, out=_ohwi(_grad_buf(w1p)))
    if wdp is not None:
        hip.conv_wgrad(px if pool else x, gs, shp(wdp), bnd[0], out=_ohwi(_grad_buf(wdp)))
    if not need_dx:
        return None
    pooled = False
    if wdp is not None:
        dxb = dgrad_auto(gs, bp.pw[3], f8, gs_slot)
        if pool:
            pooled = x.shape[1] % 2 == 0 and x.shape[2] % 2 == 0 and hip.pooled_residual_ok(dxb)
            if not pooled:
                dxb = hip.avgpool2_bwd(dxb, tuple(x.shape))
    else:
        dxb = gs
    e8 = None
    if f8 and prev_bp is not None and prev_bp.fp8 and not pooled and _fp8_dgrad_wanted(prev_bp.pw[2], x.shape, 0, True):
        e8 = fp8_slot_of(prev_bp, "_fp8_gs").emit()
    return dgrad_auto(dpre1, bp.pw[0], False, None, emit8=e8, residual=dxb, relu_mask=x if mask_x else None, residual_pooled=pooled)


class ResStageFn(torch.autograd.Function):
    @staticmethod
    def forward(ctx, x, anchor, blocks, out_grad_premasked=False, px0=None, out_spec=None):
        ctx.out_grad_premasked = out_grad_premasked
        saved, o1_8s, o2_shapes = [x], [], []
        cur = x
        for bi, bp in enumerate(blocks):
            cur, mids = _block_forward(cur, bp, True, px0 if bi == 0 else None, blocks[bi + 1].pw[0] if bi + 1 < len(blocks) else None,
                                       out_spec if bi + 1 == len(blocks) else None)
            saved += [mids[0], mids[1], mids[2], mids[3], cur]
            o1_8s += list(mids[4])
            o2_shapes.append(mids[5])
        ctx.blocks, ctx.o2_shapes = blocks, o2_shapes
        ctx.save_for_backward(*saved, *o1_8s)
        return cur

    @staticmethod
    def backward(ctx, g):
        blocks = ctx.blocks
        saved, o1_8s = ctx.saved_tensors[:-3 * len(blocks)], ctx.saved_tensors[-3 * len(blocks):]
        need_dx = ctx.needs_input_grad[0]
        gs = g.contiguous() if ctx.out_grad_premasked else hip.relu_bwd(g.contiguous(), saved[-1])
        for i in range(len(blocks) - 1, -1, -1):
            x, o1, o2, p2, px = saved[5 * i: 5 * i + 5]
            gs = _block_backward(gs, x, o1, o2, p2, px, blocks[i], need_dx or i > 0, mask_x=i > 0, prev_bp=blocks[i - 1] if i > 0 else None,
                                 c8=tuple(o1_8s[3 * i: 3 * i + 3]), o2_shape=ctx.o2_shapes[i])
        return gs, None, None, None, None, None


def _fused_stage_ok(x, blocks, out_spec):
    if os.environ.get("CDDMSL_FUSED_BOTTLENECK", "1") == "0" or out_spec is not None:
        return False
    if not (x.is_cuda and x.dtype == torch.bfloat16 and x.dim() == 4 and x.is_contiguous()):
        return False
    cin = x.shape[3]
    for bi, bp in enumerate(blocks):
        if bp.fp8 or bp.stride != 1 or any(v is None for b in bp.bn[:3] for v in b):
            return False
        if tuple(_ohwi(bp.w[0]).shape) != (64, 1, 1, cin) or tuple(_ohwi(bp.w[1]).shape) != (64, 3, 3, 64) or tuple(_ohwi(bp.w[2]).shape) != (256, 1, 1, 64):
            return False
        if bp.w[3] is not None:
            if bi > 0 or cin != 64 or tuple(_ohwi(bp.w[3]).shape) != (256, 1, 1, 64) or any(v is None for v in bp.bn[3]):
                return False
        elif cin != 256:
            return False
        cin = 256
    return bool(blocks) and bool(hip._L().cddmsl_bottleneck64_ok(x.shape[0], x.shape[1], x.shape[2], 0))


def _fused_stage_forward(x, blocks):
    T = x.dtype
    wf = lambda pw: pw.get(T, need_dgrad=False)[0]
    o1 = conv_fwd_auto(x, blocks[0].pw[0], blocks[0].bn[0][0], blocks[0].bn[0][1], False, relu=True)
    cur = x
    for bi, bp in enumerate(blocks):
        nxt = blocks[bi + 1] if bi + 1 < len(blocks) else None
        kw = dict(x0=cur, wd=wf(bp.pw[3]), bnd=bp.bn[3]) if bp.pw[3] is not None else dict(residual=cur)
        if nxt is not None:
            kw.update(w1n=wf(nxt.pw[0]), bn1n=nxt.bn[0])
        cur, o1 = hip.bottleneck64_fwd(o1, wf(bp.pw[1]), bp.bn[1], wf(bp.pw[2]), bp.bn[2], **kw)
    return cur


def res_stage(x, blocks, frozen, out_grad_premasked=False, out_spec=None):
    px0 = getattr(x, "_pooled2", None)
    if frozen or not torch.is_grad_enabled():
        if _fused_stage_ok(x, blocks, out_spec):
            return _fused_stage_forward(x, blocks)
        cur = x
        for bi, bp in enumerate(blocks):
            cur, _ = _block_forward(cur, bp, False, px0 if bi == 0 else None, blocks[bi + 1].pw[0] if bi + 1 < len(blocks) else None,
                                    out_spec if bi + 1 == len(blocks) else None)
        return cur
    return ResStageFn.apply(x, blocks[0].w[0], blocks, out_grad_premasked, px0, out_spec)


class StackHalvesFn(torch.autograd.Function):

    @staticmethod
    def forward(ctx, a, b, full):
# ... 642 lines not shown
```

### cddmsl_amd/modeling/backbone.py

```python
import os
from collections import OrderedDict

import torch
from torch import nn

from .. import hip, layers
from ..registry import BACKBONE_REGISTRY
from ..structures import ShapeSpec


def to_nhwc(x):
    v = x.permute(0, 2, 3, 1)
    return v if v.is_contiguous() else v.contiguous()


def to_nchw(x):
    return x.permute(0, 3, 1, 2)


class Conv2dW(nn.Module):

    def __init__(self, cin, cout, k):
        super().__init__()
        w = torch.empty(cout, cin, k, k).contiguous(memory_format=torch.channels_last)
# ... 125 lines not shown
    def size_divisibility(self):
        return 0

    def output_shape(self):
        return {n: ShapeSpec(channels=self._out_feature_channels[n], stride=self._out_feature_strides[n])
                for n in self._out_features}

    def freeze(self, freeze_at=0):
        assert freeze_at >= 1, "the HIP stem path has no backward: MODEL.BACKBONE.FREEZE_AT must be >= 1"
        self.freeze_at = freeze_at
        for m in (self.conv1, self.conv2, self.conv3):
            m.weight.requires_grad = False
        for idx, stage in enumerate([self.layer1, self.layer2, self.layer3, self.layer4], start=2):
            if freeze_at >= idx:
                for blk in stage:
                    blk.frozen = True
                    for p in blk.parameters():
                        p.requires_grad = False
        return self

    def _stem_weights(self, T, cp):
        dev = self.conv1.weight.device
        key = (T, cp, dev, layers.load_generation(), self.conv1.weight._version, self.conv2.weight._version, self.conv3.weight._version)
        if self._stem_w is None or self._stem_w[0] != key:
            w1 = torch.zeros(self.conv1.weight.shape[0], 3, 3, cp, device=dev)
            w1[..., :3] = self.conv1.weight.detach().permute(0, 2, 3, 1)
            ws = [hip.weight_prep(w1, None, T, True, False)[0],
                  hip.weight_prep(layers._ohwi(self.conv2.weight.detach()), None, T, True, False)[0],
                  hip.weight_prep(layers._ohwi(self.conv3.weight.detach()), None, T, True, False)[0]]
            self._stem_w = (key, ws)
        return self._stem_w[1]

    def stem_nhwc(self, x):
        w1, w2, w3 = self._stem_weights(x.dtype, x.shape[-1])
        (s1, b1), (s2, b2), (s3, b3) = self.bn1.affine(), self.bn2.affine(), self.bn3.affine()
        x = hip.conv_fwd(x, w1, s1, b1, relu=True, stride=2, pad=1)
        x = hip.conv_fwd(x, w2, s2, b2, relu=True, pad=1)
        if x.dtype == torch.bfloat16 and tuple(w3.shape) == (64, 3, 3, 32) and os.environ.get("CDDMSL_STEM_POOL", "1") != "0":
            return hip.conv3x3_pool_fwd(x, w3, s3, b3)
        x = hip.conv_fwd(x, w3, s3, b3, relu=True, pad=1)
        return hip.avgpool2_fwd(x)

    def forward_nhwc(self, x, want_res5=None, res4_spec=None):
        with torch.no_grad():
            x = self.stem_nhwc(x)
        x = self.layer1.forward_nhwc(x)
        x = self.layer2.forward_nhwc(x)
        res4 = self.layer3.forward_nhwc(x, out_spec=res4_spec)
        out = {"res4": res4}
        if "res5" in self._out_features and want_res5 is not False:
            out["res5"] = self.layer4.forward_nhwc(res4)
        return out

    def forward(self, x, want_res5=None):
        assert x.dim() == 4, f"ResNet takes an input of shape (N, C, H, W). Got {x.shape} instead!"
        T = self.compute_dtype
        cp = 8 if T == torch.bfloat16 else 4
        xin = torch.zeros(x.shape[0], x.shape[2], x.shape[3], cp, device=x.device, dtype=T)
        xin[..., :3] = x.permute(0, 2, 3, 1)
        return {k: to_nchw(v) for k, v in self.forward_nhwc(xin, want_res5).items()}


@BACKBONE_REGISTRY.register()
def build_clip_resnet_backbone(cfg, input_shape=None):
    depth = cfg.MODEL.RESNETS.DEPTH
    blocks = {50: [3, 4, 6, 3], 101: [3, 4, 23, 3], 200: [4, 6, 10, 6]}[depth]
    width = {50: 64, 101: 64, 200: 80}[depth]
    embed_dim = {50: 1024, 101: 512, 200: 640}[depth]
    res = {50: 224, 101: 224, 200: 288}[depth]
    mode = cfg.MODEL.get("COMPUTE_DTYPE", "bf16")
    dt = {"bf16": torch.bfloat16, "f32": torch.float32, "fp8": torch.bfloat16}[mode]
    net = ModifiedResNet(blocks, embed_dim, width * 32 // 64, res, width, cfg.MODEL.RESNETS.OUT_FEATURES,
                         cfg.MODEL.BACKBONE.FREEZE_AT, depth, False, True, dt)
    if mode == "fp8":
        for m in net.modules():
            if isinstance(m, Bottleneck):
                m.fp8 = True
    return net


def build_backbone(cfg, input_shape=None):
    if input_shape is None:
        input_shape = ShapeSpec(channels=len(cfg.MODEL.PIXEL_MEAN))
    return BACKBONE_REGISTRY.get(cfg.MODEL.BACKBONE.NAME)(cfg, input_shape)
```

### cddmsl_amd/modeling/rcnn.py

```python
from typing import Dict, List, Optional

import torch
import torch.distributed as dist
from torch import nn

from .. import hip, layers
from .._lib import to_device_async
from ..registry import META_ARCH_REGISTRY
from ..structures import Boxes, ImageList, Instances, as_instances
from . import resnet
from .backbone import build_backbone, to_nchw
from .clipcap import v2l
from .postprocessing import detector_postprocess
from .roi_heads import build_roi_heads
from .rpn import build_proposal_generator


class GatherLayer(torch.autograd.Function):

    @staticmethod
    def forward(ctx, input):
        ctx.save_for_backward(input)
        output = [torch.zeros_like(input) for _ in range(dist.get_world_size())]
        dist.all_gather(output, input.contiguous())
# ... 42 lines not shown
        assert not self.div_pixel or self.input_format == "RGB"
        self.use_clip_c4 = cfg.MODEL.BACKBONE.NAME == "build_clip_resnet_backbone"
        self.use_clip_attpool = cfg.MODEL.ROI_HEADS.NAME == "CLIPRes5ROIHeads" and cfg.MODEL.CLIP.USE_TEXT_EMB_CLASSIFIER
        self.projector = nn.Sequential(_Linear(768, 768), nn.ReLU(), _Linear(768, 256))
        self.compute_dtype = self.backbone.compute_dtype
        self.regions_per_image = 16
        self.region_generator = torch.Generator()
        self.share_source_pass = False
        self._shared = None
        self.defer_rpn_losses = True

    @property
    def device(self):
        return self.pixel_mean.device

    def _images(self, batched_inputs, key):
        return [x[key].to(self.device).contiguous() for x in batched_inputs]

    def preprocess_image(self, batched_inputs, key="image"):
        imgs = self._images(batched_inputs, key)
        sizes = [tuple(i.shape[-2:]) for i in imgs]
        Hp, Wp = max(s[0] for s in sizes), max(s[1] for s in sizes)
        return hip.preprocess(imgs, Hp, Wp, self.pixel_mean_list, self.pixel_std_list, self.compute_dtype, div255=self.div_pixel), sizes

    def preprocess_image_train(self, batched_inputs):
        src, tgt = self._images(batched_inputs, "image"), self._images(batched_inputs, "image_trgt")
        Hp, Wp = max(i.shape[-2] for i in src), max(i.shape[-1] for i in src)
        assert (Hp, Wp) == (max(i.shape[-2] for i in tgt), max(i.shape[-1] for i in tgt))
        return hip.preprocess224(src + tgt, Hp, Wp, self.pixel_mean_list, self.pixel_std_list, self.compute_dtype)

    def project(self, x):
        T = self.compute_dtype
        l0, l2 = self.projector[0], self.projector[2]
        h = layers.linear(x.to(T), l0.pw(), l0.bias, relu=True, out_f32=True)
        return layers.linear(h.to(T), l2.pw(), l2.bias, out_f32=True)

    def _encode(self, bb, img_nhwc):
        feats = bb.forward_nhwc(img_nhwc)
        return bb.attnpool(to_nchw(feats["res5"]))

    def v2l_contrastive(self, images_both, clipcap_model, KD_regularization=True):
        n = images_both.shape[0] // 2
        f = v2l(self._encode(self.backbone, images_both), clipcap_model)
        fs, ft = f[:n], f[n:]
        kd_loss = None
        if KD_regularization:
            with torch.no_grad():
                teacher = v2l(self._encode(self.offline_backbone, images_both[:n]), clipcap_model)
            kd_loss = torch.nn.functional.l1_loss(teacher.detach(), fs)
        p = self.project(f)
        fs, ft = gather_cat(p[:n].contiguous()), gather_cat(p[n:].contiguous())
        return layers.contrastive_loss(ft, fs), kd_loss

    def _region_level_encode(self, batched_inputs, extra_maps=None):
        n = len(batched_inputs)
        shared, self._shared = self._shared, None
        if shared is not None and not (shared["inputs"] is batched_inputs and shared["step"] == layers._STEP[0]):
            shared = None
        imgs = ([] if shared else self._images(batched_inputs, "image")) + self._images(batched_inputs, "image_trgt")
        sizes = [tuple(i.shape[-2:]) for i in self._images(batched_inputs, "image")] if shared is None else shared["sizes"]
        assert sizes == [tuple(i.shape[-2:]) for i in imgs[-n:]], "a sample and its domain twin share one geometry"
        Hp, Wp = max(s_[0] for s_ in sizes), max(s_[1] for s_ in sizes)
        x = hip.preprocess(imgs, Hp, Wp, self.pixel_mean_list, self.pixel_std_list, self.compute_dtype)
        spec = shared.get("res4_spec") if shared else None
        f = self.backbone.forward_nhwc(x, want_res5=False, res4_spec=spec)["res4"]
        gts = [as_instances(x_["instances"]).to(self.device) for x_ in batched_inputs]
        with torch.no_grad():
            if shared is None:
                props, _ = self.proposal_generator.forward_nhwc(sizes, f[:n].detach(), gts)
            else:
                if spec is not None and spec.used == 2:
                    f = layers.stack_halves(shared["res4"], f, spec.full)
                else:
                    f = torch.cat([shared["res4"], f])
                self.proposal_generator.replay_sampling_draws(shared["counts"])
                props = shared["proposals"]
            sel_cpu = [torch.randperm(len(p), generator=self.region_generator)[: self.regions_per_image] for p in props]
            offs = torch.tensor([0] + [len(p) for p in props]).cumsum(0)
            pick = to_device_async(torch.cat([s_ + int(o) for s_, o in zip(sel_cpu, offs[:-1])]), self.device)
            picked = torch.cat([p.proposal_boxes.tensor for p in props])[pick]
            props = []
            for size, b_ in zip(sizes, torch.split(picked, [len(s_) for s_ in sel_cpu])):
                inst = Instances(tuple(size))
                inst.proposal_boxes = Boxes(b_)
                props.append(inst)
        return self.roi_heads.forward_get_features_paired(f, n, props, self.backbone.layer4, self.backbone.attnpool, extra_maps)

    def forward_consistency(self, batched_inputs, clipcap_model, KD_regularization=True):
        both = self.preprocess_image_train(batched_inputs)
        n = both.shape[0] // 2
        enc_teacher = None
        if KD_regularization:
            with torch.no_grad():
                enc_teacher = self._encode(self.offline_backbone, both[:n])
        res4_img = self.backbone.forward_nhwc(both, want_res5=False)["res4"]
        pr = self.roi_heads.pooler.output_size if hasattr(self.roi_heads, "pooler") else -1
        if self.use_clip_c4 and tuple(res4_img.shape[1:3]) == (pr, pr):
            rs, rt, enc_img = self._region_level_encode(batched_inputs, extra_maps=res4_img)
        else:
            enc_img = self.backbone.attnpool(to_nchw(self.backbone.layer4.forward_nhwc(res4_img)))
            rs, rt = self._region_level_encode(batched_inputs)
        k = rs.shape[0]
        parts = [enc_img, rs, rt] + ([enc_teacher] if enc_teacher is not None else [])
        f = v2l(torch.cat(parts), clipcap_model)
        out = {}
        if enc_teacher is not None:
            out["kd_loss"] = torch.nn.functional.l1_loss(f[2 * n + 2 * k:].detach(), f[:n])
        p = self.project(f[:2 * n + 2 * k])
        out["cont_loss"] = layers.contrastive_loss(gather_cat(p[n:2 * n].contiguous()), gather_cat(p[:n].contiguous()))
        e = p[2 * n:]
        out["cont_region_loss"] = layers.contrastive_loss(gather_cat(e[:k].contiguous()), gather_cat(e[k:].contiguous()))
        return out

    @torch.no_grad()
    def inference(self, batched_inputs: List[Dict], detected_instances=None, do_postprocess: bool = True):
        assert not self.training
        images, sizes = self.preprocess_image(batched_inputs, "image")
        results = self._inference_preprocessed(images, sizes, detected_instances)
        return self._postprocess(results, batched_inputs, sizes) if do_postprocess else results

    @torch.no_grad()
    def _inference_preprocessed(self, images, sizes, detected_instances=None):
        assert not self.training
        res4 = self.backbone.forward_nhwc(images, want_res5=False)["res4"]
        feats = {"res4": to_nchw(res4)}
        if detected_instances is None:
            proposals, _ = self.proposal_generator.forward_nhwc(sizes, res4, None)
            kw = dict(res5=self.backbone.layer4, attnpool=self.backbone.attnpool) if self.use_clip_c4 else {}
            results, _ = self.roi_heads(ImageList(None, sizes), feats, proposals, None, **kw)
        else:
            results = self.roi_heads.forward_with_given_boxes(feats, [x.to(self.device) for x in detected_instances])
        return results

    @torch.no_grad()
    def inference_with_region_embeddings(self, batched_inputs: List[Dict]):
        assert not self.training
        images, sizes = self.preprocess_image(batched_inputs, "image")
        res4 = self.backbone.forward_nhwc(images, want_res5=False)["res4"]
        proposals, _ = self.proposal_generator.forward_nhwc(sizes, res4, None)
        results, embeds = self.roi_heads.inference_with_region_embeddings({"res4": to_nchw(res4)}, proposals, res5=self.backbone.layer4,
                                                                          attnpool=self.backbone.attnpool)
        for r, e in zip(results, embeds):
            r.region_embeds = e
        return self._postprocess(results, batched_inputs, sizes)

    @staticmethod
    def _postprocess(instances, batched_inputs, image_sizes):
        out = []
        for res, inp, size in zip(instances, batched_inputs, image_sizes):
            out.append({"instances": detector_postprocess(res, inp.get("height", size[0]), inp.get("width", size[1]))})
        return out

    def forward(self, batched_inputs: List[Dict], clipcap_model=None, branch="supervised", KD_regularization=True):
        if not self.training:
# ... 44 lines not shown
```

### include/cddmsl_hip.h

```cpp
#ifndef CDDMSL_HIP_H
#define CDDMSL_HIP_H
#include <stddef.h>

#ifdef __cplusplus
extern "C" {
#endif

int cddmsl_abi_version(void);

int cddmsl_conv_fwd(const void* x, const void* w, void* y, const float* scale, const float* bias, const void* residual,
                    const void* relu_mask, int Nimg, int Hi, int Wi, int Cin, int Cout, int KH, int KW, int stride, int pad,
                    int pool, int ldy, int ldr, int ldm, int relu, int out_f32, int dtype, void* stream);
int cddmsl_conv3x3_pool_fwd(const void* x, const void* w, void* y, const float* scale, const float* bias, const void* relu_mask,
                            int Nimg, int Hi, int Wi, int Cin, int Cout, int stride, int dtype, void* stream);
int cddmsl_bottleneck64_ok(int Nimg, int H, int W, int dtype);
int cddmsl_bottleneck64_fwd(const void* o1, const void* w2, const float* s2, const float* b2, const void* w3, const float* s3,
                            const float* b3, const void* residual, const void* x0, const void* wd, const float* sd,
                            const float* bd, const void* w1n, const float* s1n, const float* b1n, void* out, void* o1n,
                            int Nimg, int H, int W, int dtype, void* stream);
int cddmsl_set_workspace(void* ptr, long bytes);
int cddmsl_conv_wgrad(const void* x, const void* dy, float* dw, const float* scale, int Nimg, int Hi, int Wi, int Cin,
                      int Cout, int KH, int KW, int stride, int pad, int pool, int ldd, int dtype, void* stream);
int cddmsl_gemm_nt_batched(const void* a, const void* w, void* c, const float* bias, int M, int N, int K, int lda, int ldb, int ldc,
                           int batch, long sa, long sw, long sc, int out_f32, int dtype, void* stream);
int cddmsl_gemm_tn_batched(const void* a, const void* b, void* out, int M, int N, int K, int lda, int ldb, int ldo, int batch, long sa,
                           long sb, long so, int mode, int dtype, void* stream);
int cddmsl_last_kernel(void);
int cddmsl_plan_only(int on);
int cddmsl_weight_prep(const float* w, const float* scale, void* w_fwd, void* w_dgrad, int Cout, int KH, int KW, int Cin,
                       int dtype, void* stream);
int cddmsl_weight_prep_multi(const long long* table, int count, int dtype, void* stream);

int cddmsl_quantize_fp8(const void* x, void* y, const float* scale, float* amax, long numel, int src_dtype, void* stream);
int cddmsl_conv_fwd_fp8(const void* x, const void* w, void* y, const float* scale, const float* bias, const void* residual,
                        const void* relu_mask, int Nimg, int Hi, int Wi, int Cin, int Cout, int KH, int KW, int pad, int relu,
                        int out_f32, void* y8, const float* q8, float* amax8, void* stream);
int cddmsl_conv_fwd_q8(const void* x, const void* w, void* y, const float* scale, const float* bias, const void* residual,
                       const void* relu_mask, int Nimg, int Hi, int Wi, int Cin, int Cout, int KH, int KW, int stride, int pad,
                       int relu, void* y8, const float* q8, float* amax8, void* stream);
int cddmsl_fp8_dot_nt(const void* a, const void* b, float* c, const float* alpha, int R, int N, int K, int ldc, void* stream);
int cddmsl_conv_wgrad_fp8_ok(int Cin, int Cout, int KH, int KW, int pad, int ldd);
int cddmsl_conv_wgrad_fp8(const void* x8, const void* dy8, float* dw, const float* scale, int Nimg, int Hi, int Wi, int Cin, int Cout,
                          int KH, int KW, int pad, int ldd, void* stream);

int cddmsl_roi_align_forward(const void* x, const float* rois, void* y, void* y_pooled, int* dbg_grid, int N, int C, int H, int W,
                             int K, int ph, int pw, float spatial_scale, int sampling_ratio, int aligned, int dtype, void* stream);
int cddmsl_roi_align_backward(const void* dy, const float* rois, const int* roi_start, void* dx, float* ws_ay, float* ws_ax,
                              int* ws_fp, int N, int C, int H, int W, int K, int ph, int pw, float spatial_scale,
                              int sampling_ratio, int aligned, int dtype, void* stream);
int cddmsl_roi_align_forward_affine(const void* x, const float* rois, void* y, void* y_pooled, const float* scale,
                                    const float* bias, int relu, int N, int C, int H, int W, int K, int ph, int pw,
                                    float spatial_scale, int sampling_ratio, int aligned, int dtype, void* y8, const float* q8,
                                    float* amax8, void* stream);
int cddmsl_roi_align_backward_pooled(const void* dy, const float* rois, const int* roi_start, void* dx, float* ws_ay,
                                     float* ws_ax, int* ws_fp, int N, int C, int H, int W, int K, int ph, int pw,
                                     float spatial_scale, int sampling_ratio, int aligned, int dtype, void* stream);
int cddmsl_roi_align_nchw_anyorder(const void* input, const float* rois, void* output, int N, int C, int H, int W, int K, int ph, int pw,
                                   float spatial_scale, int sampling_ratio, int aligned, int dtype, void* temp, size_t* temp_bytes,
                                   void* stream);
int cddmsl_roi_align_backward_nchw_anyorder(const void* grad, const float* rois, void* grad_input, int N, int C, int H, int W, int K,
                                            int ph, int pw, float spatial_scale, int sampling_ratio, int aligned, int dtype, void* temp,
                                            size_t* temp_bytes, void* stream);

int cddmsl_anchors(const float* cell, float* out, int Hf, int Wf, int A, float stride, float offset, void* stream);
int cddmsl_sort_desc(const float* keys_in, float* keys_out, int* idx_scratch, int* order_out, const int* offsets, int N,
                     int total, void* temp, size_t* temp_bytes, void* stream);
int cddmsl_rpn_decode(const int* order, const float* deltas, const float* cell, const int* img_hw, float* boxes,
                      unsigned char* valid, int N, int Hf, int Wf, int A, int topk, float stride, float offset, float wx,
                      float wy, float ww, float wh, float scale_clamp, float min_size, void* stream);
int cddmsl_nms(const float* boxes, const unsigned char* valid, unsigned long long* mask_ws, int* keep, int* nkeep, int N,
               int n, float thr, int max_keep, void* stream);
int cddmsl_nms_anyorder(const float* boxes, const float* scores, long* keep, int* nkeep, int K, float iou_threshold, void* temp,
                        size_t* temp_bytes, void* stream);
int cddmsl_soft_nms(const float* boxes, const float* scores, const long* idxs, long* keep, float* keep_scores, int* nkeep, int K,
                    int method, float sigma, float iou_threshold, float prune_threshold, int max_keep, void* temp,
// ... 131 lines not shown
```

Measured before the change: 174.7.

## Fuse paired backbone passes into single conv and wgrad launches over two problems

Adds pair variants of the forward conv and weight-gradient kernels. Each launch covers two same-weight convolutions with different inputs (the full images and the crops), and the block index selects which problem a tile belongs to. The backbone runs layer2 and layer3 as paired stages, and the consistency forward uses this path when it is allowed. The aim is to cut kernel launch count and to fill the GPU better for small problems, and in wgrad the two gradients are summed in one split reduction. The cost is per-block argument selection, more template instantiations, and a more complex autograd path.

```diff
diff --git a/cddmsl_amd/csrc/conv_fwd.hip b/cddmsl_amd/csrc/conv_fwd.hip
--- a/cddmsl_amd/csrc/conv_fwd.hip
+++ b/cddmsl_amd/csrc/conv_fwd.hip
@@ -201,14 +201,16 @@
   return ((oy >> 1) < hp && (ox >> 1) < wp) ? ((long)img * hp + (oy >> 1)) * wp + (ox >> 1) : -1L;
 }
 
-template <typename T>
-__global__ __launch_bounds__(256, 2) void k_conv_fwd(ConvArgs p) {
+template <typename T, bool PAIR = false>
+__global__ __launch_bounds__(256, 2) void k_conv_fwd(typename FwdKArg<PAIR>::type q) {
   __shared__ __attribute__((aligned(16))) u32x4 lds[2][2][BM * KCH];
   const int t = threadIdx.x;
-  p.x += (long)blockIdx.y * p.bx; p.w += (long)blockIdx.y * p.bw; p.y += (long)blockIdx.y * p.by;
+  if constexpr (!PAIR) { q.x += (long)blockIdx.y * q.bx; q.w += (long)blockIdx.y * q.bw; q.y += (long)blockIdx.y * q.by; }
   const int wvu = __builtin_amdgcn_readfirstlane(t >> 6);
-  const int ntn = (p.Cout + BN - 1) / BN;
-  const int lbid = xcd_remap(blockIdx.x, gridDim.x);
+  const int ntn = (first_problem(q).Cout + BN - 1) / BN;
+  int lbid = xcd_remap(blockIdx.x, gridDim.x);
+  ConvArgs pick;
+  ConvArgs& p = pick_problem(q, pick, lbid);
   const int tile_n = lbid % ntn, tile_m = lbid / ntn;
   const int m0 = tile_m * BM, n0 = tile_n * BN;
   const int cc = t & 7, rb = t >> 3;
@@ -659,6 +661,12 @@
 
 }
 
+void launch_fwd_pair128(const ConvArgs& a, const ConvArgs& b, const Plan& p, Operand op, hipStream_t st) {
+  const ConvPairArgs q = {a, b, p.ntb};
+  if (op == OP_BF16) hipLaunchKernelGGL((k_conv_fwd<__bf16, true>), dim3(p.gx), dim3(256), 0, st, q);
+  else hipLaunchKernelGGL((k_conv_fwd<float, true>), dim3(p.gx), dim3(256), 0, st, q);
+}
+
 void launch_fwd_tile128(const ConvArgs& a, const Plan& p, Operand op, hipStream_t st) {
   if (op == OP_BF16) launch_tile128<__bf16>(a, p, st);
   else launch_tile128<float>(a, p, st);
diff --git a/cddmsl_amd/csrc/conv_fwd256.hip b/cddmsl_amd/csrc/conv_fwd256.hip
--- a/cddmsl_amd/csrc/conv_fwd256.hip
+++ b/cddmsl_amd/csrc/conv_fwd256.hip
@@ -228,18 +228,27 @@
   }
 }
 
-template <typename T, bool TAPS, bool RPOOL = false, int EPI = -1, bool PERSIST = false, bool SPLITK = false>
-__global__ __launch_bounds__(512) void k_conv_fwd256(ConvArgs p) {
+template <typename T, bool TAPS, bool RPOOL = false, int EPI = -1, bool PERSIST = false, bool SPLITK = false, bool PAIR = false>
+__global__ __launch_bounds__(512) void k_conv_fwd256(typename FwdKArg<PAIR>::type q) {
+  static_assert(!PAIR || (!RPOOL && !SPLITK), "pair launches: the plain and the persistent form");
   __shared__ __attribute__((aligned(16))) u32x4 lds[2 * 2 * 2 * 128 * KCH];
   const int t_in = threadIdx.x;
-  p.x += (long)blockIdx.y * p.bx; p.w += (long)blockIdx.y * p.bw; p.y += (long)blockIdx.y * p.by;
-  const int ntn = p.Cout >> 8;
-  const int ntiles = PERSIST ? (p.tile_limit ? p.tile_limit : ntn * ((p.M + 255) >> 8)) : 0;
-  int lbid = PERSIST ? (int)((blockIdx.x & 7) * (gridDim.x >> 3) + (blockIdx.x >> 3))
-           : SPLITK ? p.tile0 + (int)(blockIdx.x / (unsigned)p.ksplits) : xcd_remap(blockIdx.x, gridDim.x);
-  const int kt0 = SPLITK ? (int)(blockIdx.x % (unsigned)p.ksplits) * p.kper : 0;
-  if (PERSIST && lbid >= ntiles) return;
+  if constexpr (!PAIR) { q.x += (long)blockIdx.y * q.bx; q.w += (long)blockIdx.y * q.bw; q.y += (long)blockIdx.y * q.by; }
+  const ConvArgs& p0 = first_problem(q);
+  const int ntn = p0.Cout >> 8;
+  int ntiles = 0;
+  if constexpr (PERSIST) {
+    if constexpr (PAIR) ntiles = q.a.tile_limit;
+    else ntiles = p0.tile_limit ? p0.tile_limit : ntn * ((p0.M + 255) >> 8);
+  }
+  int gbid = PERSIST ? (int)((blockIdx.x & 7) * (gridDim.x >> 3) + (blockIdx.x >> 3))
+           : SPLITK ? p0.tile0 + (int)(blockIdx.x / (unsigned)p0.ksplits) : xcd_remap(blockIdx.x, gridDim.x);
+  const int kt0 = SPLITK ? (int)(blockIdx.x % (unsigned)p0.ksplits) * p0.kper : 0;
+  if (PERSIST && gbid >= ntiles) return;
   for (;;) {
+  int lbid = gbid;
+  ConvArgs pick;
+  ConvArgs& p = pick_problem(q, pick, lbid);
   int t = t_in;
   if (PERSIST) asm volatile("" : "+v"(t));
   const int lane = t & 63;
@@ -472,30 +481,32 @@
 #ifdef CDDMSL_TILE_STAMPS
   if (p.tstamps && lane == 0) {
     if (!PERSIST) asm volatile("s_waitcnt vmcnt(0)" ::: "memory");
-    unsigned long long* o = p.tstamps + ((long)(PERSIST ? lbid : (int)blockIdx.x) * 8 + wvu) * 4;
+    unsigned long long* o = p.tstamps + ((long)(PERSIST ? gbid : (int)blockIdx.x) * 8 + wvu) * 4;
     o[0] = ts_entry; o[1] = ts_loop; o[2] = ts_epi; o[3] = __builtin_amdgcn_s_memrealtime();
   }
 #endif
   if (!PERSIST) break;
-  lbid += gridDim.x;
-  if (lbid >= ntiles) break;
+  gbid += gridDim.x;
+  if (gbid >= ntiles) break;
   __builtin_amdgcn_s_barrier();
   }
 }
 
-template <typename T, bool TAPS, int EPI>
-__global__ __launch_bounds__(256, 2) void k_conv_fwd2(ConvArgs p) {
+template <typename T, bool TAPS, int EPI, bool PAIR = false>
+__global__ __launch_bounds__(256, 2) void k_conv_fwd2(typename FwdKArg<PAIR>::type q) {
   constexpr int SA = 256 * 64, SB = 128 * 64, SS = SA + SB, STAGES = 3;
   __shared__ __attribute__((aligned(16))) u32x4 lds[STAGES * SS / 16];
   const int t = threadIdx.x, lane = t & 63;
 #ifdef CDDMSL_TILE_STAMPS
   const unsigned long long ts_entry = __builtin_amdgcn_s_memrealtime();
 #endif
-  p.x += (long)blockIdx.y * p.bx; p.w += (long)blockIdx.y * p.bw; p.y += (long)blockIdx.y * p.by;
+  int lbid = xcd_remap(blockIdx.x, gridDim.x);
+  ConvArgs pick;
+  ConvArgs& p = pick_problem(q, pick, lbid);
+  if (!PAIR) { p.x += (long)blockIdx.y * p.bx; p.w += (long)blockIdx.y * p.bw; p.y += (long)blockIdx.y * p.by; }
   const int wvu = __builtin_amdgcn_readfirstlane(t >> 6);
   const int wr = wvu >> 1, wc = wvu & 1;
   const int ntn = p.Cout >> 7;
-  const int lbid = xcd_remap(blockIdx.x, gridDim.x);
   const int tile_n = lbid % ntn, tile_m = lbid / ntn;
   const int m0 = tile_m * 256, n0 = tile_n * 128;
   const int cl = (t & 3) ^ ((t >> 3) & 3);
@@ -759,6 +770,75 @@
   }
 }
 
+static TailSplit pair_tail_split(int tiles, int ntb, int ncu, int nktot, long ws_bytes) {
+  const TailSplit ts = plan_tail_split(tiles, ncu, nktot, ws_bytes);
+  return ts.rem > tiles - ntb ? TailSplit{} : ts;
+}
+
+template <typename T, bool TAPS> void launch_pair256(const ConvArgs& a, const ConvArgs& b, int ntb, int tiles, hipStream_t st, void* ws, long ws_bytes) {
+  ConvPairArgs q = {a, b, ntb};
+  const int epi = epi_of(a);
+  if constexpr (sizeof(T) == 2) {
+    if (epi >= 0) {
+      const TailSplit ts = pair_tail_split(tiles, ntb, persistent_blocks_raw(), a.Kc >> 3, ws ? ws_bytes : 0);
+      const int main_tiles = ts.splits ? tiles - ts.rem : tiles;
+      q.a.tile_limit = main_tiles;
+      bool persist = false;
+      if constexpr (!TAPS) {
+        const int nb = persistent_blocks();
+        persist = nb > 0 && main_tiles > nb && (a.Kc >> 3) <= env_int("CDDMSL_PERSIST_MAXKT", 8) && env_int("CDDMSL_PAIR_PERSIST", 1) != 0;
+        if (persist)
+          with_epi(epi, [&](auto e) { hipLaunchKernelGGL((k_conv_fwd256<T, false, false, decltype(e)::value, true, false, true>), dim3(nb), dim3(512), 0, st, q); });
+      }
+      if (!persist)
+        with_epi(epi, [&](auto e) { hipLaunchKernelGGL((k_conv_fwd256<T, TAPS, false, decltype(e)::value, false, false, true>), dim3((unsigned)main_tiles), dim3(512), 0, st, q); });
+      if (ts.splits) {
+        ConvArgs t = a;
+        t.partial = (float*)ws; t.tile0 = main_tiles - ntb; t.ksplits = ts.splits; t.kper = ts.kper;
+        hipLaunchKernelGGL((k_conv_fwd256<T, TAPS, false, -1, false, true>), dim3((unsigned)(ts.rem * ts.splits)), dim3(512), 0, st, t);
+        hipLaunchKernelGGL(k_conv_split_reduce, dim3((unsigned)(ts.rem * 64)), dim3(256), 0, st, t);
+      }
+      return;
+    }
+  }
+  hipLaunchKernelGGL((k_conv_fwd256<T, TAPS, false, -1, false, false, true>), dim3((unsigned)tiles), dim3(512), 0, st, q);
+}
+
+template <typename T, bool TAPS> void launch_pair_fwd2(const ConvArgs& a, const ConvArgs& b, int ntb, int tiles, hipStream_t st) {
+  const ConvPairArgs q = {a, b, ntb};
+  const int epi = epi_of(a);
+  if constexpr (sizeof(T) == 2) {
+    if (epi >= 0) {
+      with_epi(epi, [&](auto e) { hipLaunchKernelGGL((k_conv_fwd2<T, TAPS, decltype(e)::value, true>), dim3((unsigned)tiles), dim3(256), 0, st, q); });
+      return;
+    }
+  }
+  hipLaunchKernelGGL((k_conv_fwd2<T, TAPS, -1, true>), dim3((unsigned)tiles), dim3(256), 0, st, q);
+}
+
+template <typename T> void launch_pair_tile256(const ConvArgs& a, const ConvArgs& b, const Plan& p, hipStream_t st, void* ws, long ws_bytes) {
+  const bool taps = !(a.KH == 1 && a.KW == 1 && a.pad == 0);
+  if (p.kernel == 11) {
+    if (taps) launch_pair_fwd2<T, true>(a, b, p.ntb, (int)p.gx, st);
+    else launch_pair_fwd2<T, false>(a, b, p.ntb, (int)p.gx, st);
+  } else {
+    if (taps) launch_pair256<T, true>(a, b, p.ntb, (int)p.gx, st, ws, ws_bytes);
+    else launch_pair256<T, false>(a, b, p.ntb, (int)p.gx, st, ws, ws_bytes);
+  }
+}
+
+}
+
+extern "C" int cddmsl_pair_tail_plan(int tiles, int ntb, int ncu, int nktot, long ws_bytes, int* out) {
+  if (!out || tiles < 0 || ntb < 0 || ntb > tiles || ncu < 0 || nktot < 0 || ws_bytes < 0) return CDDMSL_ERR_ARG;
+  const TailSplit ts = pair_tail_split(tiles, ntb, ncu, nktot, ws_bytes);
+  out[0] = ts.rem; out[1] = ts.splits; out[2] = ts.kper;
+  return CDDMSL_OK;
+}
+
+void launch_fwd_pair256(const ConvArgs& a, const ConvArgs& b, const Plan& p, Operand op, hipStream_t st, void* ws, long ws_bytes) {
+  if (op == OP_BF16) launch_pair_tile256<__bf16>(a, b, p, st, ws, ws_bytes);
+  else launch_pair_tile256<float>(a, b, p, st, ws, ws_bytes);
 }
 
 void launch_fwd_tile256(const ConvArgs& a, const Plan& p, Operand op, hipStream_t st, void* ws, long ws_bytes) {
diff --git a/cddmsl_amd/csrc/conv_wgrad.hip b/cddmsl_amd/csrc/conv_wgrad.hip
--- a/cddmsl_amd/csrc/conv_wgrad.hip
+++ b/cddmsl_amd/csrc/conv_wgrad.hip
@@ -189,20 +189,24 @@
   static constexpr int MSTEP = 8;
 };
 
-template <typename T>
-__global__ __launch_bounds__(256, 2) void k_conv_wgrad_dma(WgradArgs p) {
+template <typename T, bool PAIR = false>
+__global__ __launch_bounds__(256, 2) void k_conv_wgrad_dma(typename WgradKArg<PAIR>::type q) {
   constexpr int ES = Mma<T>::ES;
   constexpr int COLS = 256 / ES;
   __shared__ __attribute__((aligned(16))) u32x4 lds[2][2][WM * 16];
   const int t = threadIdx.x, lane = t & 63, wv = t >> 6;
-  p.x += (long)blockIdx.y * p.bx; p.dy += (long)blockIdx.y * p.bd;
-  char* outp = (char*)p.dw + (long)blockIdx.y * p.bo;
+  if constexpr (!PAIR) { q.x += (long)blockIdx.y * q.bx; q.dy += (long)blockIdx.y * q.bd; }
+  const WgradArgs& p0 = first_problem(q);
+  char* outp = (char*)p0.dw + (long)blockIdx.y * p0.bo;
   const int wvu = __builtin_amdgcn_readfirstlane(t >> 6);
-  const int ntn = (p.Cout + COLS - 1) / COLS, ntk = (p.K + COLS - 1) / COLS;
+  const int ntn = (p0.Cout + COLS - 1) / COLS, ntk = (p0.K + COLS - 1) / COLS;
   int bid = xcd_remap(blockIdx.x, gridDim.x);
   const int tile_k = bid % ntk; bid /= ntk;
   const int tile_n = bid % ntn; bid /= ntn;
-  const int split = bid;
+  const int wsplit = bid;
+  int split = bid;
+  WgradArgs pick;
+  WgradArgs& p = pick_problem(q, pick, split);
   const int n0 = tile_n * COLS, k0 = tile_k * COLS;
   const int mt0 = split * p.mtiles_per_split;
   const int total_mt = (p.M + WM - 1) / WM;
@@ -301,7 +305,7 @@
 
   const int r = lane & 31, h = lane >> 5;
   if (p.ws) {
-    f32x4* dst = (f32x4*)p.ws + ((long)(split * ntn + tile_n) * ntk + tile_k) * (4 * NT * NT * 4 * 64) + (wv * NT * NT * 4) * 64 + lane;
+    f32x4* dst = (f32x4*)p.ws + ((long)(wsplit * ntn + tile_n) * ntk + tile_k) * (4 * NT * NT * 4 * 64) + (wv * NT * NT * 4) * 64 + lane;
 #pragma unroll
     for (int a = 0; a < NT; ++a)
 #pragma unroll
@@ -626,21 +630,26 @@
   }
 }
 
-__global__ __launch_bounds__(512) void k_wgrad256(WgradArgs p) {
+template <bool PAIR = false>
+__global__ __launch_bounds__(512) void k_wgrad256(typename WgradKArg<PAIR>::type q) {
   __shared__ __attribute__((aligned(16))) u32x4 lds[2 * 2 * 2 * 64 * 16];
   const int t = threadIdx.x, lane = t & 63;
 #ifdef CDDMSL_TILE_STAMPS
   const unsigned long long ts_entry = __builtin_amdgcn_s_memrealtime();
   unsigned long long ts_loop = ts_entry;
 #endif
-  p.x += (long)blockIdx.y * p.bx; p.dy += (long)blockIdx.y * p.bd;
-  char* outp = (char*)p.dw + (long)blockIdx.y * p.bo;
+  if constexpr (!PAIR) { q.x += (long)blockIdx.y * q.bx; q.dy += (long)blockIdx.y * q.bd; }
+  const WgradArgs& p0 = first_problem(q);
+  char* outp = (char*)p0.dw + (long)blockIdx.y * p0.bo;
   const int wvu = __builtin_amdgcn_readfirstlane(t >> 6);
   const int wn = wvu >> 2, wk = wvu & 3;
-  const int ntn = p.Cout >> 8, ntk = p.K >> 8;
+  const int ntn = p0.Cout >> 8, ntk = p0.K >> 8;
   int bid = xcd_remap(blockIdx.x, gridDim.x);
   const int tile_k = bid % ntk; bid /= ntk;
   const int tile_n = bid % ntn; bid /= ntn;
+  const int wsplit = bid;
+  WgradArgs pick;
+  WgradArgs& p = pick_problem(q, pick, bid);
   const int n0 = tile_n * 256, k0 = tile_k * 256;
   const int mt0 = bid * p.mtiles_per_split;
   const int nmt = min(p.mtiles_per_split, (p.M + WM - 1) / WM - mt0);
@@ -829,7 +838,7 @@
 #endif
   const int r = lane & 31, h = lane >> 5;
   if (p.ws) {
-    store_frags((f32x4*)p.ws + ((long)(bid * ntn + tile_n) * ntk + tile_k) * (8 * 32 * 64) + (wvu * 32) * 64 + lane, acc);
+    store_frags((f32x4*)p.ws + ((long)(wsplit * ntn + tile_n) * ntk + tile_k) * (8 * 32 * 64) + (wvu * 32) * 64 + lane, acc);
   } else
 #pragma unroll
   for (int a = 0; a < 4; ++a)
@@ -1071,10 +1080,26 @@
                              ntn, ntk, p.splits, a.Cout, a.K, a.ldo);
 }
 
+template <int WAVES, int FR>
+static void launch_wgrad_pair_split(void (*kernel)(WgradPairArgs), const WgradPairArgs& q, const Plan& p, hipStream_t st) {
+  constexpr int TN = WAVES == 8 ? 256 : 128, SLOTS = WAVES * FR * 64;
+  const int ntn = (q.a.Cout + TN - 1) / TN, ntk = (q.a.K + TN - 1) / TN;
+  hipLaunchKernelGGL(kernel, dim3(p.gx), dim3(WAVES * 64), 0, st, q);
+  hipLaunchKernelGGL((k_wgrad_reduce<WAVES, FR>), dim3((unsigned)(ntn * ntk * (SLOTS / 256))), dim3(256), 0, st, (const f32x4*)q.a.ws, q.a.dw, q.a.scale,
+                     ntn, ntk, p.splits, q.a.Cout, q.a.K, q.a.ldo);
+}
+void launch_wgrad_pair(const WgradArgs& a, const WgradArgs& b, const Plan& p, hipStream_t st, void* ws) {
+  WgradPairArgs q = {a, b, p.ntb};
+  q.a.ws = q.b.ws = (float*)ws;
+  q.a.mtiles_per_split = q.b.mtiles_per_split = p.mtiles_per_split;
+  if (p.kernel == 6) launch_wgrad_pair_split<8, 32>(k_wgrad256<true>, q, p, st);
+  else launch_wgrad_pair_split<4, 16>(k_conv_wgrad_dma<__bf16, true>, q, p, st);
+}
+
 void launch_wgrad(WgradArgs& a, const Plan& p, Operand op, hipStream_t st, void* ws, long ws_bytes) {
   switch (p.kernel) {
     case 12: launch_wgrad_split<8, 32>(k_wgrad256_f8, a, p, st, ws, ws_bytes); break;
-    case 6: launch_wgrad_split<8, 32>(k_wgrad256, a, p, st, ws, ws_bytes); break;
+    case 6: launch_wgrad_split<8, 32>(k_wgrad256<false>, a, p, st, ws, ws_bytes); break;
     case 5:
       if (op == OP_BF16) launch_wgrad_split<4, 16>(k_conv_wgrad_dma<__bf16>, a, p, st, ws, ws_bytes);
       else hipLaunchKernelGGL(k_conv_wgrad_dma<float>, dim3(p.gx), dim3(256), 0, st, a);
diff --git a/cddmsl_amd/csrc/gemm_common.h b/cddmsl_amd/csrc/gemm_common.h
--- a/cddmsl_amd/csrc/gemm_common.h
+++ b/cddmsl_amd/csrc/gemm_common.h
@@ -61,6 +61,28 @@
 #endif
 };
 
+struct ConvPairArgs {
+  ConvArgs a, b;
+  int ntb;
+};
+template <bool PAIR> struct FwdKArg { typedef ConvArgs type; };
+template <> struct FwdKArg<true> { typedef ConvPairArgs type; };
+__device__ __forceinline__ ConvArgs& pick_problem(ConvArgs& q, ConvArgs&, int&) { return q; }
+__device__ __forceinline__ ConvArgs& pick_problem(ConvPairArgs& q, ConvArgs& p, int& lbid) {
+  const bool second = lbid < q.ntb;
+  if (!second) lbid -= q.ntb;
+  p = q.a;
+#define CDDMSL_PICK(m) p.m = second ? q.b.m : q.a.m
+  CDDMSL_PICK(x); CDDMSL_PICK(y); CDDMSL_PICK(residual); CDDMSL_PICK(relu_mask);
+  CDDMSL_PICK(Nimg); CDDMSL_PICK(Hi); CDDMSL_PICK(Wi); CDDMSL_PICK(Ho); CDDMSL_PICK(Wo);
+  CDDMSL_PICK(ldy); CDDMSL_PICK(ldr); CDDMSL_PICK(ldm); CDDMSL_PICK(M); CDDMSL_PICK(nt_out);
+  CDDMSL_PICK(dWo.mul); CDDMSL_PICK(dWo.shr); CDDMSL_PICK(dWo.d); CDDMSL_PICK(dHo.mul); CDDMSL_PICK(dHo.shr); CDDMSL_PICK(dHo.d);
+#undef CDDMSL_PICK
+  return p;
+}
+__device__ __forceinline__ const ConvArgs& first_problem(const ConvArgs& q) { return q; }
+__device__ __forceinline__ const ConvArgs& first_problem(const ConvPairArgs& q) { return q.a; }
+
 template <typename T> struct Mma;
 template <> struct Mma<__bf16> {
   static constexpr int ES = 2;
@@ -136,6 +158,27 @@
 #endif
 };
 
+struct WgradPairArgs {
+  WgradArgs a, b;
+  int nsb;
+};
+template <bool PAIR> struct WgradKArg { typedef WgradArgs type; };
+template <> struct WgradKArg<true> { typedef WgradPairArgs type; };
+__device__ __forceinline__ WgradArgs& pick_problem(WgradArgs& q, WgradArgs&, int&) { return q; }
+__device__ __forceinline__ WgradArgs& pick_problem(WgradPairArgs& q, WgradArgs& p, int& split) {
+  const bool second = split < q.nsb;
+  if (!second) split -= q.nsb;
+  p = q.a;
+#define CDDMSL_PICK(m) p.m = second ? q.b.m : q.a.m
+  CDDMSL_PICK(x); CDDMSL_PICK(dy); CDDMSL_PICK(Nimg); CDDMSL_PICK(Hi); CDDMSL_PICK(Wi); CDDMSL_PICK(Ho); CDDMSL_PICK(Wo);
+  CDDMSL_PICK(ldd); CDDMSL_PICK(M);
+  CDDMSL_PICK(dWo.mul); CDDMSL_PICK(dWo.shr); CDDMSL_PICK(dWo.d); CDDMSL_PICK(dHo.mul); CDDMSL_PICK(dHo.shr); CDDMSL_PICK(dHo.d);
+#undef CDDMSL_PICK
+  return p;
+}
+__device__ __forceinline__ const WgradArgs& first_problem(const WgradArgs& q) { return q; }
+__device__ __forceinline__ const WgradArgs& first_problem(const WgradPairArgs& q) { return q.a; }
+
 constexpr int WM = 64;
 constexpr int WROW = 16 + 4;
 
@@ -168,6 +211,7 @@
   int splits;
   int mtiles_per_split;
   int bpb;
+  int ntb;
 };
 
 static int persistent_blocks_raw() {
@@ -185,7 +229,10 @@
 extern "C" {
 __attribute__((visibility("hidden"))) void launch_fwd_tile128(const ConvArgs& a, const Plan& p, Operand op, hipStream_t st);
 __attribute__((visibility("hidden"))) void launch_fwd_tile256(const ConvArgs& a, const Plan& p, Operand op, hipStream_t st, void* ws, long ws_bytes);
+__attribute__((visibility("hidden"))) void launch_fwd_pair128(const ConvArgs& a, const ConvArgs& b, const Plan& p, Operand op, hipStream_t st);
+__attribute__((visibility("hidden"))) void launch_fwd_pair256(const ConvArgs& a, const ConvArgs& b, const Plan& p, Operand op, hipStream_t st, void* ws, long ws_bytes);
 __attribute__((visibility("hidden"))) void launch_wgrad(WgradArgs& a, const Plan& p, Operand op, hipStream_t st, void* ws, long ws_bytes);
+__attribute__((visibility("hidden"))) void launch_wgrad_pair(const WgradArgs& a, const WgradArgs& b, const Plan& p, hipStream_t st, void* ws);
 __attribute__((visibility("hidden"))) void launch_gemm_tn(const WgradArgs& p, Operand op, const Plan& pl, int batch, int mode, hipStream_t st);
 __attribute__((visibility("hidden"))) void launch_attnpool_dx(const WgradArgs& p, unsigned gx, unsigned gy, int nbatch, int bpb, hipStream_t st);
 __attribute__((visibility("hidden"))) bool record_kernel(int id);
diff --git a/cddmsl_amd/csrc/gemm_conv.hip b/cddmsl_amd/csrc/gemm_conv.hip
--- a/cddmsl_amd/csrc/gemm_conv.hip
+++ b/cddmsl_amd/csrc/gemm_conv.hip
@@ -193,6 +193,84 @@
                       relu, out_f32, nullptr, nullptr, nullptr, stream);
 }
 
+static thread_local int g_last_pair[4] = {0, 0, 0, 0};
+
+static bool pair_legal(const ConvArgs& a, const ConvArgs& b, Operand op) {
+  if (op != OP_BF16 && op != OP_F32) return false;
+  if (a.M <= 0 || b.M <= 0) return false;
+  if (a.cpp != b.cpp || a.Kc != b.Kc || a.wrs != b.wrs || a.xrs != b.xrs || a.Cout != b.Cout || a.KH != b.KH || a.KW != b.KW ||
+      a.stride != b.stride || a.pad != b.pad || a.relu != b.relu || a.out_f32 != b.out_f32) return false;
+  if (a.y8 || b.y8 || a.pool || b.pool || a.res_pool || b.res_pool || a.res_f32 || b.res_f32 || a.pool_out || b.pool_out) return false;
+  if ((a.residual != nullptr) != (b.residual != nullptr) || (a.relu_mask != nullptr) != (b.relu_mask != nullptr)) return false;
+  const int ka = plan_fwd(a, op, 1).kernel, kb = plan_fwd(b, op, 1).kernel;
+  return (ka == 1 || ka == 3 || ka == 11) && (kb == 1 || kb == 3 || kb == 11);
+}
+
+static Plan plan_fwd_pair(const ConvArgs& a, const ConvArgs& b, Operand op) {
+  if (!pair_legal(a, b, op)) return {};
+  const long pm = (long)((a.M + 255) / 256) + (b.M + 255) / 256, pb = (b.M + 255) / 256;
+  const long m256 = env_int("CDDMSL_GEMM256", 1), m2 = env_int("CDDMSL_FWD2", 1);
+  const bool take256 = m256 != 0 && gemm256_legal(a) && gemm256_legal(b) && (m256 == 2 || (a.Cout / 256) * pm >= 160);
+  const bool take2 = m2 != 0 && fwd2_legal(a) && fwd2_legal(b) &&
+                     (m2 == 2 || (!take256 && (a.Cout / 128) * pm >= env_int("CDDMSL_FWD2_MIN", 256)));
+  Plan p = {};
+  p.gy = 1;
+  long tiles, ntb;
+  if (take2) { p.kernel = 11; tiles = (a.Cout / 128) * pm; ntb = (a.Cout / 128) * pb; }
+  else if (take256) { p.kernel = 3; tiles = (a.Cout / 256) * pm; ntb = (a.Cout / 256) * pb; }
+  else {
+    const long ntn = (a.Cout + BN - 1) / BN;
+    p.kernel = 1; tiles = ntn * ((long)((a.M + BM - 1) / BM) + (b.M + BM - 1) / BM); ntb = ntn * ((b.M + BM - 1) / BM);
+  }
+  if (tiles > 0x7fffffffL) return {};
+  p.gx = (unsigned)tiles; p.ntb = (int)ntb;
+  return p;
+}
+
+static bool aligned_to(const void* p, long n) { return ((size_t)p % (size_t)n) == 0; }
+
+extern "C" int cddmsl_conv_fwd_pair(const void* xa, void* ya, const void* residual_a, const void* relu_mask_a, int Nimg_a, int Hi_a, int Wi_a,
+                                    int ldy_a, int ldr_a, int ldm_a,
+                                    const void* xb, void* yb, const void* residual_b, const void* relu_mask_b, int Nimg_b, int Hi_b, int Wi_b,
+                                    int ldy_b, int ldr_b, int ldm_b,
+                                    const void* w, const float* scale, const float* bias, int Cin, int Cout, int KH, int KW, int stride, int pad,
+                                    int relu, int out_f32, int dtype, void* stream) {
+  g_last_pair[0] = g_last_pair[1] = g_last_pair[2] = g_last_pair[3] = 0;
+  if (dtype != 0 && dtype != 1) return CDDMSL_ERR_ARG;
+  const Operand op = (Operand)dtype;
+  const long es = elem_size(op), eso = (out_f32 & 1) ? 4 : es;
+  if (!aligned_to(w, 16) || !aligned_to(xa, 16) || !aligned_to(xb, 16) || !aligned_to(scale, 4) || !aligned_to(bias, 4)) return CDDMSL_ERR_ARG;
+  if (!aligned_to(ya, eso) || !aligned_to(yb, eso) || !aligned_to(residual_a, es) || !aligned_to(residual_b, es) ||
+      !aligned_to(relu_mask_a, es) || !aligned_to(relu_mask_b, es)) return CDDMSL_ERR_ARG;
+  ConvArgs a, b;
+  int st = fill_conv(a, op, xa, w, ya, scale, bias, residual_a, relu_mask_a, Nimg_a, Hi_a, Wi_a, Cin, Cout, KH, KW, stride, pad, 0, ldy_a, ldr_a, ldm_a,
+                     relu, out_f32, nullptr, nullptr, nullptr);
+  if (st != CDDMSL_OK) return st;
+  st = fill_conv(b, op, xb, w, yb, scale, bias, residual_b, relu_mask_b, Nimg_b, Hi_b, Wi_b, Cin, Cout, KH, KW, stride, pad, 0, ldy_b, ldr_b, ldm_b,
+                 relu, out_f32, nullptr, nullptr, nullptr);
+  if (st != CDDMSL_OK) return st;
+  auto rows16 = [&](const void* p, int ld, long e) { return !p || (ld * e) % 16 != 0 || aligned_to(p, 16); };
+  if (!rows16(ya, ldy_a, eso) || !rows16(yb, ldy_b, eso) || !rows16(residual_a, ldr_a, es) || !rows16(residual_b, ldr_b, es) ||
+      !rows16(relu_mask_a, ldm_a, es) || !rows16(relu_mask_b, ldm_b, es)) return CDDMSL_ERR_ARG;
+  const Plan pl = plan_fwd_pair(a, b, op);
+  if (pl.kernel == 0) {
+    if (a.M > 0) { st = run_fwd(a, op, plan_fwd(a, op, 1), stream); if (st != CDDMSL_OK) return st; }
+    if (b.M > 0) st = run_fwd(b, op, plan_fwd(b, op, 1), stream);
+    return st;
+  }
+  g_last_kernel = pl.kernel;
+  g_last_pair[0] = 1; g_last_pair[1] = pl.kernel; g_last_pair[2] = (int)pl.gx; g_last_pair[3] = pl.ntb;
+  if (g_plan_only) return CDDMSL_OK;
+  if (pl.kernel == 1) launch_fwd_pair128(a, b, pl, op, (hipStream_t)stream);
+  else launch_fwd_pair256(a, b, pl, op, (hipStream_t)stream, g_ws, g_ws_bytes);
+  return launch_status();
+}
+extern "C" int cddmsl_last_pair(int* out) {
+  if (!out) return CDDMSL_ERR_ARG;
+  for (int i = 0; i < 4; ++i) out[i] = g_last_pair[i];
+  return CDDMSL_OK;
+}
+
 extern "C" int cddmsl_conv3x3_pool_fwd(const void* x, const void* w, void* y, const float* scale, const float* bias, const void* relu_mask,
                                        int Nimg, int Hi, int Wi, int Cin, int Cout, int stride, int dtype, void* stream) {
   if (dtype != 0 || Cin != 32 || Cout != 64 || stride != 1 || relu_mask || !scale || !bias || Hi < 2 || Wi < 2) return CDDMSL_ERR_ARG;
@@ -358,6 +436,66 @@
   return run_wgrad(a, (Operand)dtype, plan_wgrad(a, (Operand)dtype, 1), stream);
 }
 
+static Plan plan_wgrad_pair(const WgradArgs& a, const WgradArgs& b, Operand op, long ws_bytes) {
+  if (op != OP_BF16 || a.M <= 0 || b.M <= 0 || env_int("CDDMSL_WGRAD_WS", 1) == 0) return {};
+  auto same = [](const WgradArgs& p) { return !p.pool && p.stride == 1 && p.Ho == p.Hi && p.Wo == p.Wi; };
+  if (!same(a) || !same(b)) return {};
+  const int mta = (a.M + WM - 1) / WM, mtb = (b.M + WM - 1) / WM, total_mt = mta + mtb;
+  const long tiles256 = (long)(a.Cout / 256) * (a.K / 256);
+  const long tiles = (long)((a.Cout + 127) / 128) * ((a.K + 127) / 128);
+  const long row_a = (long)a.ldd * 2 > a.xrs * 16L ? (long)a.ldd * 2 : a.xrs * 16L, row_b = (long)b.ldd * 2 > b.xrs * 16L ? (long)b.ldd * 2 : b.xrs * 16L;
+  Plan p = {};
+  p.gy = 1;
+  long tl = 0, slot_bytes = 0;
+  const long mode = env_int("CDDMSL_GEMM256", 1);
+  const bool ok256 = mode != 0 && !((a.Cout & 255) || (a.K & 255) || (a.cpp & 7) || (a.ldd & 7) || (b.ldd & 7)) &&
+                     (mode == 2 || tiles256 * total_mt >= env_int("CDDMSL_WGRAD256_MIN", 4000));
+  if (ok256) {
+    bool forced;
+    const long want = env_int("CDDMSL_WGRAD256_BLOCKS", 0, &forced);
+    const long maxs = (total_mt + 15) / 16;
+    long sp = forced ? (want + tiles256 - 1) / tiles256 : split_256_rounds(tiles256, total_mt);
+    if (sp > maxs) sp = maxs;
+    if (sp < 1) sp = 1;
+    const int mps = even_split(total_mt, &sp);
+    if (wgrad256_span_ok(mps, a.Wi, row_a) && wgrad256_span_ok(mps, b.Wi, row_b)) { p.kernel = 6; p.mtiles_per_split = mps; tl = tiles256; slot_bytes = 65536L * 4; }
+  }
+  if (!p.kernel) {
+    long sp = split_512_rounds(tiles, total_mt, !(a.KH == 1 && a.KW == 1));
+    p.kernel = 5; p.mtiles_per_split = even_split(total_mt, &sp); tl = tiles; slot_bytes = 16384L * 4;
+  }
+  const long sa = (mta + p.mtiles_per_split - 1) / p.mtiles_per_split, sb = (mtb + p.mtiles_per_split - 1) / p.mtiles_per_split;
+  const long blocks = tl * (sa + sb);
+  if (blocks > 0x7fffffffL || blocks * slot_bytes > ws_bytes) return {};
+  p.gx = (unsigned)blocks; p.splits = (int)(sa + sb); p.ntb = (int)sb;
+  return p;
+}
+
+extern "C" int cddmsl_conv_wgrad_pair(const void* xa, const void* dya, int Nimg_a, int Hi_a, int Wi_a, int ldd_a,
+                                      const void* xb, const void* dyb, int Nimg_b, int Hi_b, int Wi_b, int ldd_b,
+                                      float* dw, const float* scale, int Cin, int Cout, int KH, int KW, int stride, int pad, int dtype, void* stream) {
+  g_last_pair[0] = g_last_pair[1] = g_last_pair[2] = g_last_pair[3] = 0;
+  if (dtype != 0 && dtype != 1) return CDDMSL_ERR_ARG;
+  if (!aligned_to(xa, 16) || !aligned_to(xb, 16) || !aligned_to(dya, 16) || !aligned_to(dyb, 16) || !aligned_to(dw, 4) || !aligned_to(scale, 4)) return CDDMSL_ERR_ARG;
+  const Operand op = (Operand)dtype;
+  WgradArgs a, b;
+  int st = fill_wgrad(a, op, xa, dya, dw, scale, Nimg_a, Hi_a, Wi_a, Cin, Cout, KH, KW, stride, pad, 0, ldd_a);
+  if (st != CDDMSL_OK) return st;
+  st = fill_wgrad(b, op, xb, dyb, dw, scale, Nimg_b, Hi_b, Wi_b, Cin, Cout, KH, KW, stride, pad, 0, ldd_b);
+  if (st != CDDMSL_OK) return st;
+  const Plan pl = plan_wgrad_pair(a, b, op, g_ws ? g_ws_bytes : 0);
+  if (pl.kernel == 0) {
+    if (a.M > 0) { st = run_wgrad(a, op, plan_wgrad(a, op, 1), stream); if (st != CDDMSL_OK) return st; }
+    if (b.M > 0) st = run_wgrad(b, op, plan_wgrad(b, op, 1), stream);
+    return st;
+  }
+  g_last_kernel = pl.kernel;
+  g_last_pair[0] = 1; g_last_pair[1] = pl.kernel; g_last_pair[2] = pl.splits; g_last_pair[3] = pl.ntb;
+  if (g_plan_only) return CDDMSL_OK;
+  launch_wgrad_pair(a, b, pl, (hipStream_t)stream, g_ws);
+  return launch_status();
+}
+
 extern "C" int cddmsl_conv_wgrad_fp8_ok(int Cin, int Cout, int KH, int KW, int pad, int ldd) {
   return (Cin % 256 == 0 && Cout % 256 == 0 && KH == KW && (KH & 1) && 2 * pad == KH - 1 && ldd % 16 == 0) ? 1 : 0;
 }
diff --git a/cddmsl_amd/hip.py b/cddmsl_amd/hip.py
--- a/cddmsl_amd/hip.py
+++ b/cddmsl_amd/hip.py
@@ -23,6 +23,10 @@
         L.cddmsl_bottleneck64_ok.argtypes = [ci] * 4
         L.cddmsl_bottleneck64_fwd.argtypes = [vp] * 17 + [ci] * 4 + [vp]
         L.cddmsl_conv_wgrad.argtypes = [vp] * 4 + [ci] * 12 + [vp]
+        L.cddmsl_conv_fwd_pair.argtypes = ([vp] * 4 + [ci] * 6) * 2 + [vp] * 3 + [ci] * 9 + [vp]
+        L.cddmsl_conv_wgrad_pair.argtypes = ([vp, vp] + [ci] * 4) * 2 + [vp, vp] + [ci] * 7 + [vp]
+        L.cddmsl_last_pair.argtypes = [vp]
+        L.cddmsl_pair_tail_plan.argtypes = [ci] * 4 + [c_long, vp]
         L.cddmsl_set_workspace.argtypes = [vp, c_long]
         L.cddmsl_weight_prep.argtypes = [vp] * 4 + [ci] * 5 + [vp]
         L.cddmsl_weight_prep_multi.argtypes = [vp, ci, ci, vp]
@@ -271,6 +275,98 @@
     return y
 
 
+def _pair_chosen(launch):
+    L = _L()
+    was = L.cddmsl_plan_only(1)
+    try:
+        launch()
+    finally:
+        L.cddmsl_plan_only(was)
+    out = (ctypes.c_int * 4)()
+    L.cddmsl_last_pair(out)
+    return bool(out[0])
+
+
+def conv_fwd_pair(xa, xb, w, scale=None, bias=None, residual=(None, None), relu=False, relu_mask=(None, None), stride=1, pad=0,
+                  out_spec=None):
+    ra, rb = residual
+    ma, mb = relu_mask
+    require_cuda(xa, xb, w, scale, bias, ra, rb, ma, mb)
+    ensure_workspace(xa.device)
+    assert xa.dim() == 4 and xb.dim() == 4 and w.dim() == 4 and xa.is_contiguous() and xb.is_contiguous() and w.is_contiguous()
+    assert xa.dtype == w.dtype and xb.dtype == w.dtype
+    Cout, KH, KW, Cin = w.shape
+    assert xa.shape[3] == Cin and xb.shape[3] == Cin, (xa.shape, xb.shape, w.shape)
+    assert (ra is None) == (rb is None) and (ma is None) == (mb is None)
+    for v in (scale, bias):
+        assert v is None or (v.dtype == torch.float32 and v.numel() == Cout and v.is_contiguous())
+    (Na, Ha, Wa, _), (Nb, Hb, Wb, _) = xa.shape, xb.shape
+    Hoa, Woa = (Ha + 2 * pad - KH) // stride + 1, (Wa + 2 * pad - KW) // stride + 1
+    Hob, Wob = (Hb + 2 * pad - KH) // stride + 1, (Wb + 2 * pad - KW) // stride + 1
+    paired = _pair_chosen(lambda: _L().cddmsl_conv_fwd_pair(
+        ptr(xa), None, ptr(ra), ptr(ma), Na, Ha, Wa, Cout, Cout, Cout, ptr(xb), None, ptr(rb), ptr(mb), Nb, Hb, Wb, Cout, Cout, Cout,
+        ptr(w), ptr(scale), ptr(bias), Cin, Cout, KH, KW, stride, pad, int(relu), 0, _dt(xa), stream_ptr()))
+    if not paired:
+        return (conv_fwd(xa, w, scale, bias, ra, relu, ma, stride, pad, out_spec=out_spec),
+                conv_fwd(xb, w, scale, bias, rb, relu, mb, stride, pad))
+    if out_spec is not None and out_spec.full is None:
+        out_spec.full = torch.empty((2 * Na, Hoa, Woa, Cout), device=xa.device, dtype=xa.dtype)
+        ya, out_spec.used = out_spec.full[:Na], 1
+    elif out_spec is not None and out_spec.used == 1 and tuple(out_spec.full.shape) == (2 * Na, Hoa, Woa, Cout) and out_spec.full.dtype == xa.dtype:
+        ya, out_spec.used = out_spec.full[Na:], 2
+    else:
+        ya = torch.empty((Na, Hoa, Woa, Cout), device=xa.device, dtype=xa.dtype)
+    yb = torch.empty((Nb, Hob, Wob, Cout), device=xa.device, dtype=xa.dtype)
+    for v, y in ((ra, ya), (ma, ya), (rb, yb), (mb, yb)):
+        assert v is None or (v.dtype == xa.dtype and v.is_contiguous() and v.numel() == y.numel())
+    e0 = PROFILE.begin(name=_CONV_KERNEL.get(_L().cddmsl_last_kernel())) if PROFILE.on else None
+    st = _L().cddmsl_conv_fwd_pair(ptr(xa), ptr(ya), ptr(ra), ptr(ma), Na, Ha, Wa, Cout, Cout, Cout,
+                                   ptr(xb), ptr(yb), ptr(rb), ptr(mb), Nb, Hb, Wb, Cout, Cout, Cout,
+                                   ptr(w), ptr(scale), ptr(bias), Cin, Cout, KH, KW, stride, pad, int(relu), 0, _dt(xa), stream_ptr())
+    check(st, "cddmsl_conv_fwd_pair")
+    if e0 is not None:
+        Ma, Mb, es = Na * Hoa * Woa, Nb * Hob * Wob, xa.element_size()
+        pix = _conv_input_pixels(Na, Ha, Wa, Hoa, Woa, KH, KW, stride, False) + _conv_input_pixels(Nb, Hb, Wb, Hob, Wob, KH, KW, stride, False)
+        nops = 1 + (ra is not None) + (ma is not None)
+        PROFILE.end(e0, _CONV_KERNEL.get(_L().cddmsl_last_kernel(), "conv_fwd"), 2.0 * (Ma + Mb) * Cout * KH * KW * Cin,
+                    (Ma, Cout, KH * KW * Cin, KH, 0, stride, Mb),
+                    nbytes=float(pix * Cin * es + w.numel() * es + nops * (Ma + Mb) * Cout * es))
+    return ya, yb
+
+
+def conv_wgrad_pair(xa, dya, xb, dyb, w_shape, scale=None, pad=0, out=None):
+    require_cuda(xa, dya, xb, dyb, scale, out)
+    Cout, KH, KW, Cin = w_shape
+    assert xa.dtype == dya.dtype == xb.dtype == dyb.dtype and all(t.is_contiguous() for t in (xa, dya, xb, dyb))
+    if out is None:
+        out = torch.zeros(w_shape, device=xa.device, dtype=torch.float32)
+    assert out.dtype == torch.float32 and out.is_contiguous() and tuple(out.shape) == tuple(w_shape)
+    dims = []
+    for x, dy in ((xa, dya), (xb, dyb)):
+        N, H, W, Cin2 = x.shape
+        assert Cin == Cin2 and dy.shape[-1] == Cout and dy.numel() // Cout == N * (H + 2 * pad - KH + 1) * (W + 2 * pad - KW + 1)
+        dims.append((N, H, W))
+    ensure_workspace(xa.device)
+    (Na, Ha, Wa), (Nb, Hb, Wb) = dims
+
+    def launch():
+        return _L().cddmsl_conv_wgrad_pair(ptr(xa), ptr(dya), Na, Ha, Wa, Cout, ptr(xb), ptr(dyb), Nb, Hb, Wb, Cout,
+                                           ptr(out), ptr(scale), Cin, Cout, KH, KW, 1, pad, _dt(xa), stream_ptr())
+    if not _pair_chosen(launch):
+        conv_wgrad(xa, dya, w_shape, scale, pad=pad, out=out)
+        return conv_wgrad(xb, dyb, w_shape, scale, pad=pad, out=out)
+    e0 = PROFILE.begin(name=_CONV_KERNEL.get(_L().cddmsl_last_kernel())) if PROFILE.on else None
+    check(launch(), "cddmsl_conv_wgrad_pair")
+    if e0 is not None:
+        Ma, Mb, es = dya.numel() // Cout, dyb.numel() // Cout, xa.element_size()
+        pix = _conv_input_pixels(Na, Ha, Wa, Ha + 2 * pad - KH + 1, Wa + 2 * pad - KW + 1, KH, KW, 1, False) \
+            + _conv_input_pixels(Nb, Hb, Wb, Hb + 2 * pad - KH + 1, Wb + 2 * pad - KW + 1, KH, KW, 1, False)
+        PROFILE.end(e0, _CONV_KERNEL.get(_L().cddmsl_last_kernel(), "conv_wgrad"), 2.0 * (Ma + Mb) * Cout * KH * KW * Cin,
+                    (Ma, Cout, KH * KW * Cin, KH, 0, 1, Mb),
+                    nbytes=float(pix * Cin * es + (dya.numel() + dyb.numel()) * es + out.numel() * 4))
+    return out
+
+
 def conv3x3_pool_fwd(x, w, scale, bias, relu_mask=None, stride=1):
     require_cuda(x, w, scale, bias, relu_mask)
     assert x.dim() == 4 and w.dim() == 4 and x.is_contiguous() and w.is_contiguous() and x.dtype == w.dtype
diff --git a/cddmsl_amd/layers.py b/cddmsl_amd/layers.py
--- a/cddmsl_amd/layers.py
+++ b/cddmsl_amd/layers.py
@@ -591,6 +591,118 @@
             gs = _block_backward(gs, x, o1, o2, p2, px, blocks[i], need_dx or i > 0, mask_x=i > 0, prev_bp=blocks[i - 1] if i > 0 else None,
                                  c8=tuple(o1_8s[3 * i: 3 * i + 3]), o2_shape=ctx.o2_shapes[i])
         return gs, None, None, None, None, None
+
+
+def pair_passes_wanted(*blockss):
+    if os.environ.get("CDDMSL_PAIR_PASSES", "1") == "0" or not torch.is_grad_enabled():
+        return False
+    return all(not bp.frozen and not bp.fp8 for blocks in blockss for bp in blocks)
+
+
+def _block_forward_pair(x, bp, out_spec=None):
+    (s1, b1), (s2, b2), (s3, b3), bnd = bp.bn
+    pool = bp.stride > 1
+    T = x[0].dtype
+    wf = lambda i: bp.pw[i].get(T, need_dgrad=False)[0]
+    o1 = hip.conv_fwd_pair(x[0], x[1], wf(0), s1, b1, relu=True)
+    o2 = hip.conv_fwd_pair(o1[0], o1[1], wf(1), s2, b2, relu=True, pad=1)
+    p2, kept, px = [], [], []
+    for j in range(2):
+        if pool and _pool_bits_wanted(bp, o2[j]):
+            p, bits = hip.avgpool2_fwd_bits(o2[j])
+        else:
+            p, bits = (hip.avgpool2_fwd(o2[j]) if pool else o2[j]), None
+        p2.append(p)
+        kept.append(o2[j] if bits is None else bits)
+        px.append(hip.avgpool2_fwd(x[j]) if pool else x[j])
+    idn = hip.conv_fwd_pair(px[0], px[1], wf(3), bnd[0], bnd[1]) if bp.pw[3] is not None else x
+    out = hip.conv_fwd_pair(p2[0], p2[1], wf(2), s3, b3, residual=(idn[0], idn[1]), relu=True, out_spec=out_spec)
+    mids = tuple((o1[j], kept[j], p2[j] if pool else None, px[j] if pool else None, tuple(o2[j].shape)) for j in range(2))
+    return out, mids
+
+
+def _block_backward_pair(gs, x, o1, o2, p2, px, bp, need_dx, mask_x, o2_shape):
+    T = x[0].dtype
+    (s1, _), (s2, _), (s3, _), bnd = bp.bn
+    pool = bp.stride > 1
+    w1p, w2p, w3p, wdp = bp.w
+    shp = lambda w: _ohwi(w).shape
+    wd = lambda i: bp.pw[i].get(T, True)[1]
+    buf = lambda w: _ohwi(_grad_buf(w))
+    src3 = p2 if pool else o2
+    hip.conv_wgrad_pair(src3[0], gs[0], src3[1], gs[1], shp(w3p), s3, out=buf(w3p))
+    if pool:
+        dp2 = hip.conv_fwd_pair(gs[0], gs[1], wd(2))
+        dpre2 = tuple(hip.avgpool2_bwd_bits(dp2[j], o2_shape[j], o2[j]) if o2[j].dtype == torch.int32 else
+                      hip.avgpool2_bwd(dp2[j], o2_shape[j], mask=o2[j]) for j in range(2))
+    else:
+        dpre2 = hip.conv_fwd_pair(gs[0], gs[1], wd(2), relu_mask=(o2[0], o2[1]))
+    dpre1 = hip.conv_fwd_pair(dpre2[0], dpre2[1], wd(1), pad=1, relu_mask=(o1[0], o1[1]))
+    hip.conv_wgrad_pair(o1[0], dpre2[0], o1[1], dpre2[1], shp(w2p), s2, pad=1, out=buf(w2p))
+    hip.conv_wgrad_pair(x[0], dpre1[0], x[1], dpre1[1], shp(w1p), s1, out=buf(w1p))
+    if wdp is not None:
+        srcd = px if pool else x
+        hip.conv_wgrad_pair(srcd[0], gs[0], srcd[1], gs[1], shp(wdp), bnd[0], out=buf(wdp))
+    if not need_dx:
+        return None
+    masks = (x[0], x[1]) if mask_x else (None, None)
+    if wdp is None:
+        return hip.conv_fwd_pair(dpre1[0], dpre1[1], wd(0), residual=(gs[0], gs[1]), relu_mask=masks)
+    dxb = hip.conv_fwd_pair(gs[0], gs[1], wd(3))
+    if not pool:
+        return hip.conv_fwd_pair(dpre1[0], dpre1[1], wd(0), residual=(dxb[0], dxb[1]), relu_mask=masks)
+    pooled = [x[j].shape[1] % 2 == 0 and x[j].shape[2] % 2 == 0 and hip.pooled_residual_ok(dxb[j]) for j in range(2)]
+    if not any(pooled):
+        full = tuple(hip.avgpool2_bwd(dxb[j], tuple(x[j].shape)) for j in range(2))
+        return hip.conv_fwd_pair(dpre1[0], dpre1[1], wd(0), residual=full, relu_mask=masks)
+    return tuple(hip.conv_fwd(dpre1[j], wd(0), residual=dxb[j] if pooled[j] else hip.avgpool2_bwd(dxb[j], tuple(x[j].shape)),
+                              relu_mask=masks[j], residual_pooled=pooled[j]) for j in range(2))
+
+
+class ResStagePairFn(torch.autograd.Function):
+
+    @staticmethod
+    def forward(ctx, xa, xb, anchor, blocks, out_spec=None):
+        ctx.set_materialize_grads(False)
+        cur, saved, o2_shapes = (xa, xb), [xa, xb], []
+        for bi, bp in enumerate(blocks):
+            cur, mids = _block_forward_pair(cur, bp, out_spec if bi + 1 == len(blocks) else None)
+            for j in range(2):
+                saved += [mids[j][0], mids[j][1], mids[j][2], mids[j][3], cur[j]]
+            o2_shapes.append((mids[0][4], mids[1][4]))
+        ctx.blocks, ctx.o2_shapes = blocks, o2_shapes
+        ctx.save_for_backward(*saved)
+        return cur[0], cur[1]
+
+    @staticmethod
+    def backward(ctx, ga, gb):
+        blocks, saved = ctx.blocks, ctx.saved_tensors
+        per = lambda i, j: saved[2 + 10 * i + 5 * j: 7 + 10 * i + 5 * j]
+        xin = lambda i, j: saved[j] if i == 0 else saved[2 + 10 * (i - 1) + 5 * j + 4]
+        n = len(blocks)
+        if ga is None or gb is None:
+            j = 0 if gb is None else 1
+            g = ga if j == 0 else gb
+            if g is None:
+                return None, None, None, None, None
+            need_dx = ctx.needs_input_grad[j]
+            gs = hip.relu_bwd(g.contiguous(), saved[-6 if j == 0 else -1])
+            for i in range(n - 1, -1, -1):
+                o1, o2, p2, px, _ = per(i, j)
+                gs = _block_backward(gs, xin(i, j), o1, o2, p2, px, blocks[i], need_dx or i > 0, mask_x=i > 0,
+                                     prev_bp=blocks[i - 1] if i > 0 else None, o2_shape=ctx.o2_shapes[i][j])
+            return (gs if j == 0 else None), (gs if j == 1 else None), None, None, None
+        need_dx = ctx.needs_input_grad[0] or ctx.needs_input_grad[1]
+        gs = (hip.relu_bwd(ga.contiguous(), saved[-6]), hip.relu_bwd(gb.contiguous(), saved[-1]))
+        for i in range(n - 1, -1, -1):
+            ma, mb = per(i, 0), per(i, 1)
+            gs = _block_backward_pair(gs, (xin(i, 0), xin(i, 1)), (ma[0], mb[0]), (ma[1], mb[1]), (ma[2], mb[2]), (ma[3], mb[3]), blocks[i],
+                                      need_dx or i > 0, mask_x=i > 0, o2_shape=ctx.o2_shapes[i])
+        return (gs[0] if gs is not None else None), (gs[1] if gs is not None else None), None, None, None
+
+
+def res_stage_pair(xa, xb, blocks, out_spec=None):
+    return ResStagePairFn.apply(xa, xb, blocks[0].w[0], blocks, out_spec)
 
 
 def _fused_stage_ok(x, blocks, out_spec):
diff --git a/cddmsl_amd/modeling/backbone.py b/cddmsl_amd/modeling/backbone.py
--- a/cddmsl_amd/modeling/backbone.py
+++ b/cddmsl_amd/modeling/backbone.py
@@ -201,6 +201,18 @@
             out["res5"] = self.layer4.forward_nhwc(res4)
         return out
 
+    def pair_passes_ok(self):
+        return layers.pair_passes_wanted(self.layer2.block_params(), self.layer3.block_params())
+
+    def forward_nhwc_pair(self, x_images, x_crops, res4_spec=None):
+        xs = []
+        for x in (x_images, x_crops):
+            with torch.no_grad():
+                x = self.stem_nhwc(x)
+            xs.append(self.layer1.forward_nhwc(x))
+        xa, xb = layers.res_stage_pair(xs[0], xs[1], self.layer2.block_params())
+        return layers.res_stage_pair(xa, xb, self.layer3.block_params(), out_spec=res4_spec)
+
     def forward(self, x, want_res5=None):
         assert x.dim() == 4, f"ResNet takes an input of shape (N, C, H, W). Got {x.shape} instead!"
         T = self.compute_dtype
diff --git a/cddmsl_amd/modeling/rcnn.py b/cddmsl_amd/modeling/rcnn.py
--- a/cddmsl_amd/modeling/rcnn.py
+++ b/cddmsl_amd/modeling/rcnn.py
@@ -118,7 +118,7 @@
         fs, ft = gather_cat(p[:n].contiguous()), gather_cat(p[n:].contiguous())
         return layers.contrastive_loss(ft, fs), kd_loss
 
-    def _region_level_encode(self, batched_inputs, extra_maps=None):
+    def _region_level_encode(self, batched_inputs, extra_maps=None, crops=None):
         n = len(batched_inputs)
         shared, self._shared = self._shared, None
         if shared is not None and not (shared["inputs"] is batched_inputs and shared["step"] == layers._STEP[0]):
@@ -129,7 +129,10 @@
         Hp, Wp = max(s_[0] for s_ in sizes), max(s_[1] for s_ in sizes)
         x = hip.preprocess(imgs, Hp, Wp, self.pixel_mean_list, self.pixel_std_list, self.compute_dtype)
         spec = shared.get("res4_spec") if shared else None
-        f = self.backbone.forward_nhwc(x, want_res5=False, res4_spec=spec)["res4"]
+        if crops is not None:
+            f, extra_maps = self.backbone.forward_nhwc_pair(x, crops, res4_spec=spec)
+        else:
+            f = self.backbone.forward_nhwc(x, want_res5=False, res4_spec=spec)["res4"]
         gts = [as_instances(x_["instances"]).to(self.device) for x_ in batched_inputs]
         with torch.no_grad():
             if shared is None:
@@ -150,6 +153,10 @@
                 inst = Instances(tuple(size))
                 inst.proposal_boxes = Boxes(b_)
                 props.append(inst)
+        pr = self.roi_heads.pooler.output_size if hasattr(self.roi_heads, "pooler") else -1
+        if crops is not None and tuple(extra_maps.shape[1:3]) != (pr, pr):
+            rs, rt = self.roi_heads.forward_get_features_paired(f, n, props, self.backbone.layer4, self.backbone.attnpool, None)
+            return rs, rt, self.backbone.attnpool(to_nchw(self.backbone.layer4.forward_nhwc(extra_maps)))
         return self.roi_heads.forward_get_features_paired(f, n, props, self.backbone.layer4, self.backbone.attnpool, extra_maps)
 
     def forward_consistency(self, batched_inputs, clipcap_model, KD_regularization=True):
@@ -159,13 +166,16 @@
         if KD_regularization:
             with torch.no_grad():
                 enc_teacher = self._encode(self.offline_backbone, both[:n])
-        res4_img = self.backbone.forward_nhwc(both, want_res5=False)["res4"]
-        pr = self.roi_heads.pooler.output_size if hasattr(self.roi_heads, "pooler") else -1
-        if self.use_clip_c4 and tuple(res4_img.shape[1:3]) == (pr, pr):
-            rs, rt, enc_img = self._region_level_encode(batched_inputs, extra_maps=res4_img)
-        else:
-            enc_img = self.backbone.attnpool(to_nchw(self.backbone.layer4.forward_nhwc(res4_img)))
-            rs, rt = self._region_level_encode(batched_inputs)
+        if self.use_clip_c4 and hasattr(self.backbone, "forward_nhwc_pair") and self.backbone.pair_passes_ok():
+            rs, rt, enc_img = self._region_level_encode(batched_inputs, crops=both)
+        else:
+            res4_img = self.backbone.forward_nhwc(both, want_res5=False)["res4"]
+            pr = self.roi_heads.pooler.output_size if hasattr(self.roi_heads, "pooler") else -1
+            if self.use_clip_c4 and tuple(res4_img.shape[1:3]) == (pr, pr):
+                rs, rt, enc_img = self._region_level_encode(batched_inputs, extra_maps=res4_img)
+            else:
+                enc_img = self.backbone.attnpool(to_nchw(self.backbone.layer4.forward_nhwc(res4_img)))
+                rs, rt = self._region_level_encode(batched_inputs)
         k = rs.shape[0]
         parts = [enc_img, rs, rt] + ([enc_teacher] if enc_teacher is not None else [])
         f = v2l(torch.cat(parts), clipcap_model)
diff --git a/include/cddmsl_hip.h b/include/cddmsl_hip.h
--- a/include/cddmsl_hip.h
+++ b/include/cddmsl_hip.h
@@ -21,6 +21,16 @@
 int cddmsl_set_workspace(void* ptr, long bytes);
 int cddmsl_conv_wgrad(const void* x, const void* dy, float* dw, const float* scale, int Nimg, int Hi, int Wi, int Cin,
                       int Cout, int KH, int KW, int stride, int pad, int pool, int ldd, int dtype, void* stream);
+int cddmsl_conv_fwd_pair(const void* xa, void* ya, const void* residual_a, const void* relu_mask_a, int Nimg_a, int Hi_a, int Wi_a,
+                         int ldy_a, int ldr_a, int ldm_a, const void* xb, void* yb, const void* residual_b, const void* relu_mask_b,
+                         int Nimg_b, int Hi_b, int Wi_b, int ldy_b, int ldr_b, int ldm_b, const void* w, const float* scale,
+                         const float* bias, int Cin, int Cout, int KH, int KW, int stride, int pad, int relu, int out_f32, int dtype,
+                         void* stream);
+int cddmsl_conv_wgrad_pair(const void* xa, const void* dya, int Nimg_a, int Hi_a, int Wi_a, int ldd_a, const void* xb, const void* dyb,
+                           int Nimg_b, int Hi_b, int Wi_b, int ldd_b, float* dw, const float* scale, int Cin, int Cout, int KH, int KW,
+                           int stride, int pad, int dtype, void* stream);
+int cddmsl_last_pair(int* out);
+int cddmsl_pair_tail_plan(int tiles, int ntb, int ncu, int nktot, long ws_bytes, int* out);
 int cddmsl_gemm_nt_batched(const void* a, const void* w, void* c, const float* bias, int M, int N, int K, int lda, int ldb, int ldc,
                            int batch, long sa, long sw, long sc, int out_f32, int dtype, void* stream);
 int cddmsl_gemm_tn_batched(const void* a, const void* b, void* out, int M, int N, int K, int lda, int ldb, int ldo, int batch, long sa,
```

Result: no change. 176.1 (median of 6 runs) (+0.8%).
